# minh86/ModelCrowdNav

Measured on AMD Instinct MI355X. Metric: env-steps/sec (whole node), 5-human CrowdSim x batched envs, higher is better.
Workload: dtype f64

## Files before the change

### modelcrowdnav_amd/csrc/env_rollout_quad.hip

```cpp
#include <hip/hip_runtime.h>
#include <stdint.h>
#include "../../include/mcn.h"
#include "quad_common.hpp"
#include "env_step_params.hpp"
#include "env_common.hpp"

namespace mcn {
void note_dispatch(const char *family);
void note_rollout_form(int form);

#ifdef MCN_DIAG
#define MCN_STAMP_SLOTS 64
#define MCN_STAMP_WAVES 8192
__device__ unsigned long long g_stamps[MCN_STAMP_WAVES * MCN_STAMP_SLOTS];
#define STAMP(slot)                                                                                              \
    do {                                                                                                         \
        const int w_ = blockIdx.x * (blockDim.x >> 6) + (threadIdx.x >> 6);                                      \
        if ((threadIdx.x & 63) == 0 && (slot) < MCN_STAMP_SLOTS && w_ < MCN_STAMP_WAVES)                         \
            g_stamps[w_ * MCN_STAMP_SLOTS + (slot)] = __builtin_amdgcn_s_memrealtime();                          \
    } while (0)
#define STAMP_WHERE()                                                                                            \
    do {                                                                                                         \
        const int w_ = blockIdx.x * (blockDim.x >> 6) + (threadIdx.x >> 6);                                      \
        if ((threadIdx.x & 63) == 0 && w_ < MCN_STAMP_WAVES)                                                     \
            g_stamps[w_ * MCN_STAMP_SLOTS + 38] =                                                                \
                (unsigned long long)__builtin_amdgcn_s_getreg((4) | (0 << 6) | (31 << 11)) |                     \
                ((unsigned long long)__builtin_amdgcn_s_getreg((20) | (0 << 6) | (31 << 11)) << 32);             \
    } while (0)
int read_counts(void *dst, size_t bytes, int reset)
{
    if (bytes > sizeof(g_diag_counts)) bytes = sizeof(g_diag_counts);
    const int rc = hipMemcpyFromSymbol(dst, HIP_SYMBOL(g_diag_counts), bytes) == hipSuccess ? (int)(bytes / 4) : -1;
    if (reset) {
        void *sym = nullptr;
        if (hipGetSymbolAddress(&sym, HIP_SYMBOL(g_diag_counts)) == hipSuccess) (void)hipMemset(sym, 0, sizeof(g_diag_counts));
    }
    return rc;
}
int read_stamps(void *dst, size_t bytes)
{
    if (bytes > sizeof(g_stamps)) bytes = sizeof(g_stamps);
    return hipMemcpyFromSymbol(dst, HIP_SYMBOL(g_stamps), bytes) == hipSuccess ? (int)(bytes / 8) : -1;
}
#else
#define STAMP(slot)
#define STAMP_WHERE()
#endif

__device__ __forceinline__ int bperm_i(int byte_addr, int v) { return __builtin_amdgcn_ds_bpermute(byte_addr, v); }
__device__ __forceinline__ float bperm_f(int byte_addr, float v)
{
    return __builtin_bit_cast(float, bperm_i(byte_addr, __builtin_bit_cast(int, v)));
}
__device__ __forceinline__ double bperm_d(int byte_addr, double v)
{
    const long long b = __builtin_bit_cast(long long, v);
    const int lo = bperm_i(byte_addr, (int)b), hi = bperm_i(byte_addr, (int)(b >> 32));
    return __builtin_bit_cast(double, ((long long)hi << 32) | (unsigned int)lo);
}

template <class V>
__device__ __forceinline__ V in_vgpr(V v)
{
    asm volatile("" : "+v"(v));
    return v;
}

typedef const __attribute__((address_space(4))) StepParams *KernargPtr;
__device__ __forceinline__ KernargPtr kernarg_here()
{
    KernargPtr q = (KernargPtr)__builtin_amdgcn_kernarg_segment_ptr();
    asm volatile("" : "+s"(q));
    return q;
}

template <int NT>
struct Wg4 {
    static_assert(NT == 5, "the four-wavefront form is built for 5 humans only");
    static constexpr int EW = 8;
    static constexpr int NQ = EW * NT;
};

template <int CTRL>
__device__ __forceinline__ int dpp_i(int v) { return __builtin_amdgcn_mov_dpp(v, CTRL, 0xf, 0xf, true); }
template <int CTRL>
__device__ __forceinline__ double dpp_d(double v)
{
    const long long b = __builtin_bit_cast(long long, v);
    const int lo = dpp_i<CTRL>((int)b), hi = dpp_i<CTRL>((int)(b >> 32));
    return __builtin_bit_cast(double, ((long long)hi << 32) | (unsigned int)lo);
}
constexpr int DPP_QUAD_XOR1 = 0xB1, DPP_QUAD_XOR2 = 0x4E, DPP_ROW_HALF_MIRROR = 0x141;

template <int NT, int VIS, bool UNI>
__device__ __forceinline__ void rollout_wg4(const StepParams &p, const int T)
{
    static_assert(VIS == 0, "the four-wavefront form is built for an invisible robot only");
    constexpr int EW = Wg4<NT>::EW, NQ = Wg4<NT>::NQ;
    __shared__ float4 s_pack[NQ];
    __shared__ float2 s_res[2 * NQ], s_inv[NQ];
    __shared__ double2 s_hpos[NQ];
    __shared__ double s_hrad[NQ];
    STAMP(0);
    STAMP_WHERE();
#ifdef MCN_DIAG
    if (p.debug_noop) return;
#endif
    const int tid = threadIdx.x;
    const int role = __builtin_amdgcn_readfirstlane(tid >> 6);
    const unsigned nb_ = gridDim.x, xcd_ = blockIdx.x & 7u, idx_ = blockIdx.x >> 3;
    const unsigned qq_ = nb_ >> 3, rr__ = nb_ & 7u;
    const unsigned chunk_ = (xcd_ < rr__ ? xcd_ * (qq_ + 1) : rr__ * (qq_ + 1) + (xcd_ - rr__) * qq_) + idx_;
    const mcn_env_cfg &c = p.cfg;
    const mcn_rollout &ro = p.roll;

    if (role < 3) {
        const int lane = tid & 63, k = tid & 3, q = tid >> 2;
        const bool pop = q < NQ;
        const int ge = q / NT, h = q - ge * NT;
        const bool active = pop && (long)chunk_ * EW + ge < p.E;
        const int hi = pop ? q : 0;
        const bool cand_h = k < NT - 1;
        const int j = cand_h ? k + (k >= h ? 1 : 0) : h;
        const int ci = pop ? ge * NT + j : 0;
        const bool publish = pop && k == 0;
        const float inv_th = in_vgpr(1.0f / c.orca_time_horizon), inv_ts = in_vgpr(1.0f / (float)c.time_step);
        int rd_h = hi + NQ, rd_c = ci + NQ;
        __syncthreads();
        STAMP(1);

        for (int t = 0; t < T; ++t) {
            float4 P = s_pack[hi];
            float2 cp = *reinterpret_cast<const float2 *>(s_pack + ci);
            float2 v = s_res[rd_h], cv = s_res[rd_c];
            float2 fm = s_inv[hi];
            float orad = s_inv[ci].x;
            asm volatile("" : "+v"(P.x), "+v"(P.y), "+v"(P.z), "+v"(P.w), "+v"(cp.x), "+v"(cp.y), "+v"(v.x), "+v"(v.y),
                              "+v"(cv.x), "+v"(cv.y), "+v"(fm.x), "+v"(fm.y), "+v"(orad));
            float rx, ry;
            quad_orca_core(c, lane, k, cand_h && active, make_float4(P.x, P.y, v.x, v.y), make_float4(P.z, P.w, fm.x, fm.y),
                           make_float4(cp.x, cp.y, cv.x, cv.y), orad, inv_th, inv_ts, rx, ry);
            if (publish) s_res[(t & 1) * NQ + hi] = make_float2(rx, ry);
            rd_h = in_vgpr(hi + (t & 1) * NQ); rd_c = in_vgpr(ci + (t & 1) * NQ);
            if (t < 20) STAMP(40 + t);
            __syncthreads();
            __syncthreads();
            if (t < 37) STAMP(2 + t);
        }
    } else {
        static_assert(EW * 8 == 64, "eight lanes per env fill the wavefront");
        const double dt = in_vgpr(c.time_step);
        const bool do_reset = p.has_roll && ro.pool_hpos != nullptr;
        const int l = tid & 63;
        const int g = l >> 3, h = l & 7;
        const bool pop = h < NT;
        const int hs = g * NT + (pop ? h : 0);
        const long e = (long)chunk_ * EW + g;
        const bool active = pop && e < p.E;
        const long eb = e < p.E ? e : 0;
        const long a = eb * NT + (pop ? h : 0);
        const bool lead = active && h == 0;
        constexpr bool unicycle = UNI;
        const bool has_state = p.has_roll && ro.state != nullptr;
        const bool track = c.track_human_times && p.st.human_times != nullptr;

        double2 pos = reinterpret_cast<const double2 *>(p.st.hpos)[a];
        double2 vel = reinterpret_cast<const double2 *>(p.st.hvel)[a];
        double2 goal = reinterpret_cast<const double2 *>(p.st.hgoal)[a];
        double rad = p.st.hrad[a];
        double vpref = p.st.hvpref[a];
        double htime = p.st.human_times ? p.st.human_times[a] : 0.0;
        double hax = 0, hay = 0;
        double2 rpos = reinterpret_cast<const double2 *>(p.st.rpos)[eb];
        double2 rvel = reinterpret_cast<const double2 *>(p.st.rvel)[eb];
        double2 rgoal = reinterpret_cast<const double2 *>(p.st.rgoal)[eb];
        const double rrad = p.st.rrad[eb];
        double gtime = p.st.gtime[eb];
        double rtheta = p.st.rtheta ? p.st.rtheta[eb] : 0.0;
        mcn_roll_rec rs = {0, 0, 0, 0, 0, 0};
        if (has_state) rs = ro.state[eb];
        const double2 *act_ptr = reinterpret_cast<const double2 *>(p.actions) + eb;
        const long act_stride = in_vgpr((long)p.E);
        const double *disc_table = in_vgpr(ro.disc_table);
        const int disc_last = in_vgpr(ro.disc_len - 1);
        const bool has_theta = p.st.rtheta != nullptr;
        double2 act_next = *act_ptr;
        double o_rew = 0, o_dmin = 0;
        int o_dn = 0, o_inf = 0, o_hh = 0;
        const double k_timeout_at = in_vgpr(c.time_limit - 1);
        const double k_collision = in_vgpr(c.collision_penalty), k_success = in_vgpr(c.success_reward);
        const double k_discomfort = in_vgpr(c.discomfort_dist), k_factor = in_vgpr(c.discomfort_penalty_factor);
        const int k_stride = ro.case_stride, k_pool = ro.pool_size;
        const bool count_hh = c.count_hh != 0;
        {
            float4 A, B;
            quad_orca_operands(c, pos, vel, goal, rad, vpref, A, B);
            if (pop) {
                s_pack[hs] = make_float4(A.x, A.y, B.x, B.y); s_res[NQ + hs] = make_float2(A.z, A.w);
                s_inv[hs] = make_float2(B.z, B.w);
                s_hpos[hs] = pos; s_hrad[hs] = rad;
            }
        }
        __syncthreads();
        STAMP(1);

        for (int t = 0; t < T; ++t) {
            const double2 act = act_next;
            act_ptr += act_stride;
            if (t + 1 < T) act_next = *act_ptr;
            double ep_disc = 0;
            if (has_state) ep_disc = disc_table[rs.ep_steps < disc_last ? rs.ep_steps : disc_last];

            double2 eff = act;
            if (unicycle) {
                eff.x = act.x * cos(act.y + rtheta);
                eff.y = act.x * sin(act.y + rtheta);
            }
            double cd;
            {
                const double px = pos.x - rpos.x, py = pos.y - rpos.y;
                const double vx = vel.x - eff.x, vy = vel.y - eff.y;
                cd = p2s_origin(px, py, px + vx * dt, py + vy * dt) - rad - rrad;
            }
            cd = pop ? cd : INFINITY;
            int hh = 0;
            {
                static_assert(NT / 2 == 2, "two pairs per lane");
                double s2[2], ra[2], rb[2];
                bool near_any = false;
                const bool counted = active & count_hh;
#pragma unroll
                for (int d = 1; d <= NT / 2; ++d) {
                    const int jj = h + d >= NT ? h + d - NT : h + d;
                    const int pi = g * NT + (pop ? jj : 0);
                    const double2 ppos = s_hpos[pi];
                    const double prad = s_hrad[pi];
                    ra[d - 1] = jj > h ? rad : prad; rb[d - 1] = jj > h ? prad : rad;
                    const double dx = pos.x - ppos.x, dy = pos.y - ppos.y;
                    s2[d - 1] = dx * dx + dy * dy;
                    const double reach = ra[d - 1] + rb[d - 1] + 1e-6;
                    near_any |= counted & (s2[d - 1] < reach * reach);
                }
                if (__any(near_any)) {
                    DIAG_COUNT(2);
#pragma unroll
                    for (int d = 0; d < NT / 2; ++d)
                        hh += (counted & ((sqrt(s2[d]) - ra[d] - rb[d]) < 0)) ? 1 : 0;
                }
            }
            double dmin = cd;
            int hh_sum = hh;
            dmin = fmin(dmin, dpp_d<DPP_QUAD_XOR1>(dmin));       hh_sum += dpp_i<DPP_QUAD_XOR1>(hh_sum);
            dmin = fmin(dmin, dpp_d<DPP_QUAD_XOR2>(dmin));       hh_sum += dpp_i<DPP_QUAD_XOR2>(hh_sum);
            dmin = fmin(dmin, dpp_d<DPP_ROW_HALF_MIRROR>(dmin)); hh_sum += dpp_i<DPP_ROW_HALF_MIRROR>(hh_sum);

            double endx, endy, new_theta = rtheta, nrvx, nrvy;
            if (unicycle) {
                const double th = rtheta + act.y;
                endx = rpos.x + cos(th) * act.x * dt;
                endy = rpos.y + sin(th) * act.x * dt;
                new_theta = pymod(rtheta + act.y, 2 * M_PI);
                nrvx = act.x * cos(new_theta); nrvy = act.x * sin(new_theta);
            } else {
                endx = rpos.x + act.x * dt; endy = rpos.y + act.y * dt;
                nrvx = act.x; nrvy = act.y;
            }
            bool reaching = false;
            {
                const double gx = endx - rgoal.x, gy = endy - rgoal.y, near = rrad + 1e-6;
                if (__any(gx * gx + gy * gy < near * near)) DIAG_COUNT(3);
                if (__any(gx * gx + gy * gy < near * near)) reaching = norm2(gx, gy) < rrad;
            }
            double rew; int inf, dn;
            if (gtime >= k_timeout_at)          { rew = 0; dn = 1; inf = MCN_INFO_TIMEOUT; }
            else if (dmin < 0)                  { rew = k_collision; dn = 1; inf = MCN_INFO_COLLISION; }
            else if (reaching)                  { rew = k_success; dn = 1; inf = MCN_INFO_REACHGOAL; }
            else if (dmin < k_discomfort)       { rew = (dmin - k_discomfort) * k_factor * dt; dn = 0; inf = MCN_INFO_DANGER; }
            else                                { rew = 0; dn = 0; inf = MCN_INFO_NOTHING; }
            o_rew = rew; o_dmin = dmin; o_dn = dn; o_inf = inf; o_hh = hh_sum;
            const double t_new = gtime + dt;

            const int case_g = rs.next_case;
            if (has_state) {
                bool danger = inf == MCN_INFO_DANGER;
                if (danger) {
                    const KernargPtr kp = kernarg_here();
                    const int lim = kp->roll.danger_episodes, sf = kp->roll.danger_short_from;
                    danger = lim <= 0 || rs.fin_count < lim - ((sf > 0 && e >= sf - 1) ? 1 : 0);
                }
                rs.danger_count += danger ? 1 : 0;
                rs.danger_dist_sum = danger ? rs.danger_dist_sum + dmin : rs.danger_dist_sum;
                const double ret = rs.ep_return + ep_disc * rew;
                if (lead && dn) {
                    const int kf = rs.fin_count;
                    const KernargPtr kp = kernarg_here();
                    const int fin_slots = kp->roll.fin_slots;
                    double *fin_return = kp->roll.fin_return, *fin_time = kp->roll.fin_time;
                    uint8_t *fin_info = kp->roll.fin_info;
                    const bool keep = (fin_slots == 1) || (kf < fin_slots);
                    const long rec = (long)(fin_slots == 1 ? 0 : kf) * kp->E + e;
                    if (keep && fin_return) fin_return[rec] = ret;
                    if (keep && fin_time)   fin_time[rec] = (inf == MCN_INFO_TIMEOUT) ? kp->cfg.time_limit : t_new;
                    if (keep && fin_info)   fin_info[rec] = (uint8_t)inf;
                }
                rs.fin_count += dn;
                rs.ep_return = dn ? 0.0 : ret;
                rs.ep_steps = dn ? 0 : rs.ep_steps + 1;
                if (do_reset) {
                    int nc = rs.next_case + k_stride;
                    nc = nc >= k_pool ? nc - k_pool : nc;
                    rs.next_case = dn ? nc : rs.next_case;
                }
            }

            if (do_reset && dn) {
                const KernargPtr kp = kernarg_here();
                const double k_theta0 = kp->roll.robot_theta0;
                rpos = make_double2(kp->roll.robot_start[0], kp->roll.robot_start[1]);
                rgoal = make_double2(kp->roll.robot_goal[0], kp->roll.robot_goal[1]);
                rvel = make_double2(0, 0);
                if (has_theta) rtheta = k_theta0;
                gtime = 0;
            } else {
                rpos = make_double2(endx, endy);
                rvel = make_double2(nrvx, nrvy);
                if (unicycle) rtheta = new_theta;
                gtime = t_new;
            }

            const bool restart = do_reset && dn;
            float4 n_pack = make_float4(0, 0, 0, 0);
            float2 n_fvel = make_float2(0, 0), n_inv = make_float2(0, 0);
            if (restart) {
                DIAG_COUNT(1);
                if (active) {
                    const long pa = (long)case_g * NT + h;
                    const KernargPtr kp = kernarg_here();
                    const double2 *pool_hvel = reinterpret_cast<const double2 *>(kp->roll.pool_hvel);
                    vel = make_double2(0, 0);
                    if (pool_hvel) vel = pool_hvel[pa];
                    pos = reinterpret_cast<const double2 *>(kp->roll.pool_hpos)[pa];
                    goal = reinterpret_cast<const double2 *>(kp->roll.pool_hgoal)[pa];
                    rad = kp->roll.pool_hrad[pa];
                    vpref = kp->roll.pool_hvpref[pa];
                }
                htime = 0;
                float4 A, B;
                quad_orca_operands(c, pos, vel, goal, rad, vpref, A, B);
                n_pack = make_float4(in_vgpr(A.x), in_vgpr(A.y), in_vgpr(B.x), in_vgpr(B.y));
                n_fvel = make_float2(in_vgpr(A.z), in_vgpr(A.w));
                n_inv = make_float2(in_vgpr(B.z), in_vgpr(B.w));
            }
            const bool any_restart = __any(restart);

            if (t < 20) STAMP(40 + t);
            __syncthreads();
            float2 *vel_io = s_res + (t & 1) * NQ;
            {
                const float2 r = vel_io[hs];
                hax = (double)r.x; hay = (double)r.y;
            }
            if (!restart) {
                pos = make_double2(pos.x + hax * dt, pos.y + hay * dt);
                if (pop) s_pack[hs] = quad_orca_position_pack(pos, goal);
            }
            if (any_restart) {
                if (pop && restart) { s_pack[hs] = n_pack; vel_io[hs] = n_fvel; s_inv[hs] = n_inv; }
            }
            __syncthreads();
            if (t < 37) STAMP(2 + t);

            if (pop) s_hpos[hs] = pos;
            if (!restart) {
                vel = make_double2(hax, hay);
                if (track && htime == 0 && norm2(pos.x - goal.x, pos.y - goal.y) < rad) htime = t_new;
            }
            if (any_restart) {
                if (pop && restart) s_hrad[hs] = rad;
            }
        }

        long a2 = a, e2 = e;
        asm volatile("" : "+v"(a2), "+v"(e2));
        const KernargPtr kp = kernarg_here();
        if (active) {
            reinterpret_cast<double2 *>(kp->st.hpos)[a2] = pos;
            reinterpret_cast<double2 *>(kp->st.hvel)[a2] = vel;
            if (do_reset) {
                reinterpret_cast<double2 *>(kp->st.hgoal)[a2] = goal;
                kp->st.hrad[a2] = rad;
                kp->st.hvpref[a2] = vpref;
            }
            double *human_times = kp->st.human_times, *human_act = kp->out.human_act;
            if (human_times) human_times[a2] = htime;
            if (human_act) reinterpret_cast<double2 *>(human_act)[a2] = make_double2(hax, hay);
        }
        if (lead) {
            reinterpret_cast<double2 *>(kp->st.rpos)[e2] = rpos;
            reinterpret_cast<double2 *>(kp->st.rvel)[e2] = rvel;
            if (do_reset) reinterpret_cast<double2 *>(kp->st.rgoal)[e2] = rgoal;
            double *rth = kp->st.rtheta;
            if (rth) rth[e2] = rtheta;
            kp->st.gtime[e2] = gtime;
            store_step_rec(kp->out.rec + e2, o_rew, o_dmin, o_dn, o_inf, o_hh);
            if (has_state) kp->roll.state[e2] = rs;
        }
    }
    STAMP(39);
}

template <int NT, int VIS, bool UNI>
__global__ __launch_bounds__(256, 2) void env_rollout_wg4_kernel(const StepParams p, const int T)
{
    rollout_wg4<NT, VIS, UNI>(p, T);
}

template <int NT, int VIS, bool UNI, bool SPLIT>
__global__ __launch_bounds__(SPLIT ? 128 : 64, SPLIT ? 3 : 1) void env_rollout_quad_kernel(const StepParams p, const int T)
{
    __shared__ double2 s_hpos[16], s_hvel[16], s_rpos[16], s_rvel[16];
    __shared__ double s_hrad[16];
    __shared__ int s_dn[16], s_case[16];
    STAMP(0);
    STAMP_WHERE();
#ifdef MCN_DIAG
    if (p.debug_noop) return;
#endif
    const int role = SPLIT ? (int)(threadIdx.x >> 6) : -1;
    const bool do_orca = role != 1, do_pair = role != 0;
    constexpr int NC = NT - 1 + VIS;
    constexpr int LPE = 4 * NT;
    constexpr int G = 64 / LPE;
    static_assert(NC >= 0 && NC <= 4, "quad kernel handles at most 4 ORCA neighbours");
    const int lane = threadIdx.x & 63;
    const int g = lane / LPE;
    const int r = lane - g * LPE;
    const int h = r >> 2, k = r & 3;
#ifndef MCN_QUAD_XCD
#define MCN_QUAD_XCD 1
#endif
    const unsigned nb_ = gridDim.x, xcd_ = blockIdx.x & 7u, idx_ = blockIdx.x >> 3;
    const unsigned qq_ = nb_ >> 3, rr__ = nb_ & 7u;
    const unsigned chunk_ = MCN_QUAD_XCD ? (xcd_ < rr__ ? xcd_ * (qq_ + 1) : rr__ * (qq_ + 1) + (xcd_ - rr__) * qq_) + idx_
                                         : blockIdx.x;
    const long e = (long)chunk_ * G + g;
    const bool active = (g < G) && (e < p.E);
    const long eb = active ? e : 0;
    const long a = eb * NT + h;
    const int gi = g < G ? g : 0;
    const int hi = g < G ? g * NT + h : 0;
    const mcn_env_cfg &c = p.cfg;
    const mcn_rollout &ro = p.roll;
    const double dt = in_vgpr(c.time_step);
    const bool lead = active && r == 0 && do_pair;
    const bool hlead = active && k == 0 && do_orca;
    constexpr bool unicycle = UNI;
    const bool has_state = p.has_roll && ro.state != nullptr;
    const bool do_reset = p.has_roll && ro.pool_hpos != nullptr;
    const bool track = c.track_human_times && p.st.human_times != nullptr;

    double2 pos = reinterpret_cast<const double2 *>(p.st.hpos)[a];
    double2 vel = reinterpret_cast<const double2 *>(p.st.hvel)[a];
    double2 goal = reinterpret_cast<const double2 *>(p.st.hgoal)[a];
    double rad = p.st.hrad[a];
    double vpref = p.st.hvpref[a];
    double htime = p.st.human_times ? p.st.human_times[a] : 0.0;
    double2 rpos = reinterpret_cast<const double2 *>(p.st.rpos)[eb];
    double2 rvel = reinterpret_cast<const double2 *>(p.st.rvel)[eb];
    double2 rgoal = reinterpret_cast<const double2 *>(p.st.rgoal)[eb];
    const double rrad = p.st.rrad[eb];
    double gtime = p.st.gtime[eb];
    double rtheta = p.st.rtheta ? p.st.rtheta[eb] : 0.0;
    mcn_roll_rec rs = {0, 0, 0, 0, 0, 0};
    if (has_state) rs = ro.state[eb];

    const bool cand_h = k < NT - 1;
    const bool cand_r = VIS && (k == NT - 1);
    const int j = cand_h ? k + (k >= h ? 1 : 0) : h;
    const int l0 = lane - r;
    const int src = ((l0 + 4 * j) & 63) << 2;

    const double2 *act_ptr = reinterpret_cast<const double2 *>(p.actions) + eb;
    const long act_stride = in_vgpr((long)p.E);
    const double *disc_table = in_vgpr(ro.disc_table);
    const int disc_last = in_vgpr(ro.disc_len - 1);
    const bool has_theta = p.st.rtheta != nullptr;
    double2 act_next = *act_ptr;
    double o_rew = 0, o_dmin = 0;
    int o_dn = 0, o_inf = 0, o_hh = 0;
    double hax = 0, hay = 0;
    const float inv_th = in_vgpr(1.0f / c.orca_time_horizon), inv_ts = in_vgpr(1.0f / (float)c.time_step);
    STAMP(1);

    for (int t = 0; t < T; ++t) {
        const double2 act = act_next;
        act_ptr += act_stride;
        if (do_pair && t + 1 < T) act_next = *act_ptr;
        double ep_disc = 0;
        if (do_pair && has_state) ep_disc = disc_table[rs.ep_steps < disc_last ? rs.ep_steps : disc_last];

        double2 cpos;
        cpos.x = bperm_d(src, pos.x);
        cpos.y = bperm_d(src, pos.y);
        double crd = bperm_d(src, rad);
        float cvx = bperm_f(src, (float)vel.x), cvy = bperm_f(src, (float)vel.y);
        if (cand_r) { cpos = rpos; crd = rrad; }

        int dn = 0, case_g = 0;
        double t_new = 0;

        if (do_orca) {
            if (cand_r) { cvx = (float)rvel.x; cvy = (float)rvel.y; }
            float rx, ry;
            quad_orca_velocity(c, lane, k, (cand_h || cand_r) && active, pos, vel, goal, rad, vpref,
                               make_float4((float)cpos.x, (float)cpos.y, cvx, cvy), crd, inv_th, inv_ts, rx, ry);
            hax = (double)rx; hay = (double)ry;
        }

        if (do_pair) {
            double2 eff = act;
            if (unicycle) {
                eff.x = act.x * cos(act.y + rtheta);
                eff.y = act.x * sin(act.y + rtheta);
            }
            double cd;
            {
                const double px = pos.x - rpos.x, py = pos.y - rpos.y;
                const double vx = vel.x - eff.x, vy = vel.y - eff.y;
                cd = p2s_origin(px, py, px + vx * dt, py + vy * dt) - rad - rrad;
            }
            int hh = 0;
            {
                const double dx = pos.x - cpos.x, dy = pos.y - cpos.y;
                const bool counted = active & (c.count_hh != 0) & cand_h & (j > h);
                const double s2 = dx * dx + dy * dy, reach = rad + crd + 1e-6;
                if (__any(counted & (s2 < reach * reach))) DIAG_COUNT(2);
                if (__any(counted & (s2 < reach * reach)))
                    hh = (counted & ((sqrt(s2) - rad - crd) < 0)) ? 1 : 0;
            }
            hh += __builtin_amdgcn_update_dpp(0, hh, 0xB1, 0xf, 0xf, false);
            hh += __builtin_amdgcn_update_dpp(0, hh, 0x4E, 0xf, 0xf, false);
            double dmin = INFINITY;
            int hh_sum = 0;
#pragma unroll
            for (int q = 0; q < NT; ++q) {
                const int s = (l0 + 4 * q) & 63;
                dmin = fmin(dmin, __shfl(cd, s));
                hh_sum += __shfl(hh, s);
            }

            double endx, endy, new_theta = rtheta, nrvx, nrvy;
            if (unicycle) {
                const double th = rtheta + act.y;
                endx = rpos.x + cos(th) * act.x * dt;
                endy = rpos.y + sin(th) * act.x * dt;
                new_theta = pymod(rtheta + act.y, 2 * M_PI);
                nrvx = act.x * cos(new_theta); nrvy = act.x * sin(new_theta);
            } else {
                endx = rpos.x + act.x * dt; endy = rpos.y + act.y * dt;
                nrvx = act.x; nrvy = act.y;
            }
            bool reaching = false;
            {
                const double gx = endx - rgoal.x, gy = endy - rgoal.y, near = rrad + 1e-6;
                if (__any(gx * gx + gy * gy < near * near)) DIAG_COUNT(3);
                if (__any(gx * gx + gy * gy < near * near)) reaching = norm2(gx, gy) < rrad;
            }
            const KernargPtr kc = kernarg_here();
            const double k_time_limit = kc->cfg.time_limit, k_timeout_at = k_time_limit - 1;
            const double k_collision = kc->cfg.collision_penalty, k_success = kc->cfg.success_reward;
            const double k_discomfort = kc->cfg.discomfort_dist, k_factor = kc->cfg.discomfort_penalty_factor;
            double rew; int inf;
            if (gtime >= k_timeout_at)          { rew = 0; dn = 1; inf = MCN_INFO_TIMEOUT; }
            else if (dmin < 0)                  { rew = k_collision; dn = 1; inf = MCN_INFO_COLLISION; }
            else if (reaching)                  { rew = k_success; dn = 1; inf = MCN_INFO_REACHGOAL; }
            else if (dmin < k_discomfort)       { rew = (dmin - k_discomfort) * k_factor * dt; dn = 0; inf = MCN_INFO_DANGER; }
            else                                { rew = 0; dn = 0; inf = MCN_INFO_NOTHING; }
            o_rew = rew; o_dmin = dmin; o_dn = dn; o_inf = inf; o_hh = hh_sum;
            t_new = gtime + dt;

            case_g = rs.next_case;
            if (has_state) {
                bool danger = inf == MCN_INFO_DANGER;
                if (danger) {
                    const KernargPtr kp = kernarg_here();
                    const int lim = kp->roll.danger_episodes, sf = kp->roll.danger_short_from;
                    danger = lim <= 0 || rs.fin_count < lim - ((sf > 0 && e >= sf - 1) ? 1 : 0);
                }
                rs.danger_count += danger ? 1 : 0;
                rs.danger_dist_sum = danger ? rs.danger_dist_sum + dmin : rs.danger_dist_sum;
                const double ret = rs.ep_return + ep_disc * rew;
                if (lead && dn) {
                    const int kf = rs.fin_count;
                    const KernargPtr kp = kernarg_here();
                    const int fin_slots = kp->roll.fin_slots;
                    double *fin_return = kp->roll.fin_return, *fin_time = kp->roll.fin_time;
                    uint8_t *fin_info = kp->roll.fin_info;
                    const bool keep = (fin_slots == 1) || (kf < fin_slots);
                    const long rec = (long)(fin_slots == 1 ? 0 : kf) * kp->E + e;
                    if (keep && fin_return) fin_return[rec] = ret;
                    if (keep && fin_time)   fin_time[rec] = (inf == MCN_INFO_TIMEOUT) ? k_time_limit : t_new;
                    if (keep && fin_info)   fin_info[rec] = (uint8_t)inf;
                }
                rs.fin_count += dn;
                rs.ep_return = dn ? 0.0 : ret;
                rs.ep_steps = dn ? 0 : rs.ep_steps + 1;
                if (do_reset) {
                    const int k_stride = kc->roll.case_stride, k_pool = kc->roll.pool_size;
                    int nc = rs.next_case + k_stride;
                    nc = nc >= k_pool ? nc - k_pool : nc;
                    rs.next_case = dn ? nc : rs.next_case;
                }
            }

            if (do_reset && dn) {
                const KernargPtr kp = kernarg_here();
                const double k_theta0 = kp->roll.robot_theta0;
                rpos = make_double2(kp->roll.robot_start[0], kp->roll.robot_start[1]);
                rgoal = make_double2(kp->roll.robot_goal[0], kp->roll.robot_goal[1]);
                rvel = make_double2(0, 0);
                if (has_theta) rtheta = k_theta0;
                gtime = 0;
            } else {
                rpos = make_double2(endx, endy);
                rvel = make_double2(nrvx, nrvy);
                if (unicycle) rtheta = new_theta;
                gtime = t_new;
            }
        }

        if (SPLIT) {
            if (lead) {
                s_dn[gi] = dn; s_case[gi] = case_g;
                if (VIS) { s_rpos[gi] = rpos; s_rvel[gi] = rvel; }
            }
            __syncthreads();
            if (role == 0) {
                dn = s_dn[gi]; case_g = s_case[gi];
                if (VIS) { rpos = s_rpos[gi]; rvel = s_rvel[gi]; }
            }
        }

        if (do_orca) {
            if (do_reset && dn) {
                DIAG_COUNT(1);
                if (active) {
                    const long pa = (long)case_g * NT + h;
                    const KernargPtr kp = kernarg_here();
                    const double2 *pool_hvel = reinterpret_cast<const double2 *>(kp->roll.pool_hvel);
                    pos = reinterpret_cast<const double2 *>(kp->roll.pool_hpos)[pa];
                    goal = reinterpret_cast<const double2 *>(kp->roll.pool_hgoal)[pa];
                    rad = kp->roll.pool_hrad[pa];
                    vpref = kp->roll.pool_hvpref[pa];
                    vel = pool_hvel ? pool_hvel[pa] : make_double2(0, 0);
                }
                htime = 0;
            } else {
                pos = make_double2(pos.x + hax * dt, pos.y + hay * dt);
                vel = make_double2(hax, hay);
                if (track && htime == 0 && norm2(pos.x - goal.x, pos.y - goal.y) < rad) htime = SPLIT ? gtime + dt : t_new;
            }
        }
        if (SPLIT) {
            if (role == 0) gtime = (do_reset && dn) ? 0.0 : gtime + dt;
            if (hlead) { s_hpos[hi] = pos; s_hvel[hi] = vel; s_hrad[hi] = rad; }
            __syncthreads();
            if (role == 1) { pos = s_hpos[hi]; vel = s_hvel[hi]; rad = s_hrad[hi]; }
        }
        if (t < 37) STAMP(2 + t);
    }

    {
        long a2 = a, e2 = e;
        asm volatile("" : "+v"(a2), "+v"(e2));
        const KernargPtr kp = kernarg_here();
        if (hlead) {
            reinterpret_cast<double2 *>(kp->st.hpos)[a2] = pos;
            reinterpret_cast<double2 *>(kp->st.hvel)[a2] = vel;
            if (do_reset) {
                reinterpret_cast<double2 *>(kp->st.hgoal)[a2] = goal;
                kp->st.hrad[a2] = rad;
                kp->st.hvpref[a2] = vpref;
            }
            double *human_times = kp->st.human_times, *human_act = kp->out.human_act;
            if (human_times) human_times[a2] = htime;
            if (human_act) reinterpret_cast<double2 *>(human_act)[a2] = make_double2(hax, hay);
        }
        if (lead) {
            reinterpret_cast<double2 *>(kp->st.rpos)[e2] = rpos;
            reinterpret_cast<double2 *>(kp->st.rvel)[e2] = rvel;
            if (do_reset) reinterpret_cast<double2 *>(kp->st.rgoal)[e2] = rgoal;
            double *rth = kp->st.rtheta;
            if (rth) rth[e2] = rtheta;
            kp->st.gtime[e2] = gtime;
            store_step_rec(kp->out.rec + e2, o_rew, o_dmin, o_dn, o_inf, o_hh);
            if (has_state) kp->roll.state[e2] = rs;
        }
    }
    STAMP(39);
}

template <int NT, int VIS, bool UNI>
static void launch_rollout_kin(const StepParams &p, int T, int blocks, hipStream_t stream)
{
    if constexpr (NT == 5 && VIS == 0) {
        if (p.quad_split == 2) {
            constexpr int EW = Wg4<NT>::EW;
            hipLaunchKernelGGL((env_rollout_wg4_kernel<NT, VIS, UNI>), dim3((p.E + EW - 1) / EW), dim3(256), 0, stream, p, T);
            note_rollout_form(2);
            return;
        }
    }
    if (p.quad_split)
        hipLaunchKernelGGL((env_rollout_quad_kernel<NT, VIS, UNI, true>), dim3(blocks), dim3(128), 0, stream, p, T);
    else
        hipLaunchKernelGGL((env_rollout_quad_kernel<NT, VIS, UNI, false>), dim3(blocks), dim3(64), 0, stream, p, T);
    note_rollout_form(p.quad_split ? 1 : 0);
}

template <int NT, int VIS>
static void launch_rollout_one(const StepParams &p, int T, hipStream_t stream)
{
    constexpr int G = 64 / (4 * NT);
    const int blocks = (p.E + G - 1) / G;
    if (p.cfg.robot_kinematics == MCN_KIN_UNICYCLE)
        launch_rollout_kin<NT, VIS, true>(p, T, blocks, stream);
    else
        launch_rollout_kin<NT, VIS, false>(p, T, blocks, stream);
}

bool launch_env_rollout_quad(const StepParams &p, int T, hipStream_t stream)
{
    if (p.cfg.human_policy != MCN_HUMANS_ORCA || p.cfg.orca_max_neighbors < 4 || !p.update) return false;
    const int vis = p.cfg.robot_visible ? 1 : 0;
    const int nc = p.N - 1 + vis;
    if (nc > 4 || p.N < 1) return false;
    switch (p.N * 2 + vis) {
        case 2:  launch_rollout_one<1, 0>(p, T, stream); break;
        case 3:  launch_rollout_one<1, 1>(p, T, stream); break;
        case 4:  launch_rollout_one<2, 0>(p, T, stream); break;
        case 5:  launch_rollout_one<2, 1>(p, T, stream); break;
        case 6:  launch_rollout_one<3, 0>(p, T, stream); break;
        case 7:  launch_rollout_one<3, 1>(p, T, stream); break;
        case 8:  launch_rollout_one<4, 0>(p, T, stream); break;
        case 9:  launch_rollout_one<4, 1>(p, T, stream); break;
        case 10: launch_rollout_one<5, 0>(p, T, stream); break;
        default: return false;
    }
    note_dispatch("env_rollout_quad_kernel");
    return true;
}

}
```

### modelcrowdnav_amd/csrc/mcn_api.hip

```cpp
#include <hip/hip_runtime.h>
#include <string.h>
#include <stdlib.h>
#include <math.h>
#include <mutex>
#include "../../include/mcn.h"

#include "env_step_params.hpp"
#include "lp3_queue.hpp"

namespace mcn {
int launch_env_step(const StepParams &p, hipStream_t stream);
bool launch_env_rollout_quad(const StepParams &p, int T, hipStream_t stream);
bool launch_env_step_loop(const StepParams &p, int T, hipStream_t stream);
bool launch_env_step_loop_sf(const StepParams &p, int T, hipStream_t stream);
int launch_env_step_loop_orca(const StepParams &p, const ClosedLoop &cl, int T, hipStream_t stream);
int launch_scenario_pool(const mcn_scenario_cfg &c, uint64_t seed, int64_t first_case, int P, int N, double *hpos,
                         double *hgoal, double *hrad, double *hvpref, hipStream_t stream);
struct SarlParams;
long sarl_workspace_float4s(int E, int N, int A);
int launch_mlp_world(const mcn_mlp_world_net *net, const double *hpos, const double *hvel, double *out_vel, int E, int N,
                     hipStream_t stream);
int launch_attn_world(const mcn_attn_world_net *net, const double *hpos, const double *hvel, const int32_t *hcount,
                      void *workspace, double *out_vel, int E, int N, hipStream_t stream);
long attn_world_workspace_float4s(int E, int N);
int launch_sarl_c(const mcn_sarl_net *net, const mcn_env_state *st, const double *actions, int A, double dt,
                  double gamma_pow, int kinematics, void *workspace, double *values, int32_t *best, double *best_val,
                  float *attention, const double *next_hpos, const double *next_hvel, const double *reward_in,
                  double *action_out, double epsilon, unsigned long long seed, int E, int N, const float *om_init,
                  hipStream_t stream);
int launch_sarl_om(const mcn_env_state *st, double dt, const double *next_hpos, const double *next_hvel,
                   double cell_size, const float *w_om, const float *b_om, float *om, float *init, int E, int N,
                   hipStream_t stream);
int launch_lstm_rl(const mcn_lstm_rl_net *net, const mcn_env_state *st, const double *actions, int A, double dt,
                   double gamma_pow, int kinematics, double *values, int32_t *best, double *best_val, int32_t *order,
                   const double *next_hpos, const double *next_hvel, const double *reward_in, double *action_out,
                   double epsilon, unsigned long long seed, int E, int N, hipStream_t stream);
int launch_cadrl(const mcn_cadrl_net *net, const mcn_env_state *st, const double *actions, int A, double dt,
                 double gamma_pow, int kinematics, double *values, int32_t *best, double *best_val,
                 const double *next_hpos, const double *next_hvel, const double *reward_in, double *action_out,
                 double epsilon, unsigned long long seed, int E, int N, hipStream_t stream);
int launch_lstm_rl_order(const double *hpos, const double *rpos, const int32_t *hcount, int32_t *order, int E, int N,
                         hipStream_t stream);
#ifdef MCN_DIAG
int read_pool_clock(void *dst, size_t bytes);
int read_sarl_phases(void *dst, size_t bytes, int reset);
#endif
int launch_sgan(const mcn_sgan_net *net, double *hist, int push_slot, int oldest, const double *cur_pos,
                const float *noise, const int32_t *hcount, void *workspace, double *out_vel, float *out_rel,
                double time_step, int E, int N, hipStream_t stream);
int launch_sgan_predict(const mcn_sgan_net *net, const double *hist, int oldest, const float *noise, int K, int T,
                        const int32_t *hcount, void *workspace, float *out_rel, double *out_pos, int E, int N,
                        hipStream_t stream);
int launch_orca_batch(const float *self, const float *others, const int32_t *n_other, float *out,
                      int B, int M, float neighbor_dist, int max_neighbors, float time_horizon, float time_step,
                      hipStream_t stream);
int launch_orca_finish(const mcn_env_state &st, float *sim_vel, const uint8_t *select, int max_steps, int32_t *steps,
                       float *traj, double time_step, float neighbor_dist, int max_neighbors, float time_horizon,
                       int E, int N, hipStream_t stream);
#ifdef MCN_DIAG
int read_stamps(void *dst, size_t bytes);
int read_counts(void *dst, size_t bytes, int reset);
#endif
}

static mcn_tuning g_tuning;
static bool g_tuning_init = false;
static std::mutex g_tuning_mu;
static int env_or(const char *name, int dflt)
{
    const char *v = getenv(name);
    return v ? atoi(v) : dflt;
}
static mcn_tuning tuning_from_env()
{
    mcn_tuning t;
    memset(&t, 0, sizeof(t));
    t.force_generic = env_or("MCN_FORCE_GENERIC", 0);
    t.quad_max_envs = env_or("MCN_QUAD_MAX_ENVS", -1);
    t.quad_split = env_or("MCN_QUAD_SPLIT", -1);
    t.rollout_fused = env_or("MCN_ROLLOUT_FUSED", -1);
    t.rollout_split = env_or("MCN_ROLLOUT_SPLIT", -1);
    t.step_block = env_or("MCN_STEP_BLOCK", -1);
    t.pair_stream = env_or("MCN_PAIR_STREAM", -1);
    t.lp3_defer = env_or("MCN_LP3_DEFER", -1);
    t.sarl_x3 = env_or("MCN_SARL_X3", -1);
    return t;
}
static mcn_tuning tuning()
{
    std::lock_guard<std::mutex> lock(g_tuning_mu);
    if (!g_tuning_init) { g_tuning = tuning_from_env(); g_tuning_init = true; }
    return g_tuning;
}

namespace mcn { bool tuning_sarl_x3() { return tuning().sarl_x3 != 0; } }

static uint16_t bf16_rne(float x)
{
    uint32_t u;
    memcpy(&u, &x, 4);
    if ((u & 0x7fffffffu) > 0x7f800000u) return (uint16_t)((u >> 16) | 0x40);
    u += 0x7fffu + ((u >> 16) & 1u);
    return (uint16_t)(u >> 16);
}
static float bf16_to_f32(uint16_t h) { const uint32_t u = (uint32_t)h << 16; float f; memcpy(&f, &u, 4); return f; }

int64_t mcn_pack_x3_bytes(int32_t NT, int32_t KT)
{
    if (NT <= 0 || KT <= 0) return 0;
    return (int64_t)NT * ((KT + 1) / 2) * 3 * 64 * 8 * 2;
}

int mcn_pack_x3(const float *wfrag, int32_t NT, int32_t KT, void *x3_out)
{
    if (!wfrag || !x3_out || NT <= 0 || KT <= 0) return MCN_EINVAL;
    const int KB = (KT + 1) / 2;
    uint16_t *out = reinterpret_cast<uint16_t *>(x3_out);
    for (int n = 0; n < NT; ++n)
        for (int m = 0; m < KB; ++m)
            for (int lane = 0; lane < 64; ++lane)
                for (int s = 0; s < 8; ++s) {
                    const int t = 2 * m + (s >> 2);
                    const float w = t < KT ? wfrag[(((size_t)n * KT + t) * 64 + lane) * 4 + (s & 3)] : 0.0f;
                    const uint16_t hi = bf16_rne(w);
                    const float r1 = w - bf16_to_f32(hi);
                    const uint16_t mid = bf16_rne(r1);
                    const float r2 = r1 - bf16_to_f32(mid);
                    const size_t at = (((size_t)n * KB + m) * 3 * 64 + lane) * 8 + s;
                    out[at] = hi; out[at + 64 * 8] = mid; out[at + 2 * 64 * 8] = bf16_rne(r2);
                }
    return MCN_OK;
}

static thread_local const char *g_last_dispatch = "";
namespace mcn { void note_dispatch(const char *family) { g_last_dispatch = family; } }
const char *mcn_last_dispatch(void) { return g_last_dispatch; }
static thread_local int32_t g_last_rollout_form = -1;
namespace mcn { void note_rollout_form(int form) { g_last_rollout_form = form; } }
int32_t mcn_last_rollout_form(void) { return g_last_rollout_form; }

int32_t mcn_abi_version(void) { return MCN_ABI_VERSION; }
int64_t mcn_sizeof(int32_t which)
{
    switch (which) {
        case MCN_SIZEOF_ENV_CFG: return sizeof(mcn_env_cfg);
        case MCN_SIZEOF_ENV_STATE: return sizeof(mcn_env_state);
        case MCN_SIZEOF_ENV_OUT: return sizeof(mcn_env_out);
        case MCN_SIZEOF_ROLLOUT: return sizeof(mcn_rollout);
        case MCN_SIZEOF_TUNING: return sizeof(mcn_tuning);
        case MCN_SIZEOF_STEP_REC: return sizeof(mcn_step_rec);
        case MCN_SIZEOF_ROLL_REC: return sizeof(mcn_roll_rec);
        case MCN_SIZEOF_SARL_NET: return sizeof(mcn_sarl_net);
        case MCN_SIZEOF_SGAN_NET: return sizeof(mcn_sgan_net);
        case MCN_SIZEOF_SCENARIO_CFG: return sizeof(mcn_scenario_cfg);
        case MCN_SIZEOF_MLP_WORLD_NET: return sizeof(mcn_mlp_world_net);
        case MCN_SIZEOF_ATTN_WORLD_NET: return sizeof(mcn_attn_world_net);
        case MCN_SIZEOF_SARL_X3: return sizeof(mcn_sarl_x3);
        case MCN_SIZEOF_LSTM_RL_NET: return sizeof(mcn_lstm_rl_net);
        case MCN_SIZEOF_CADRL_NET: return sizeof(mcn_cadrl_net);
        default: return -1;
    }
}

static int fill_step_params(mcn::StepParams &p, const mcn_env_cfg *cfg, const mcn_env_state *st, const double *actions,
                            const double *given_v, const mcn_env_out *out, const mcn_rollout *roll,
                            int32_t E, int32_t N, int32_t update, bool social_force = false, bool needs_actions = true)
{
    if (!cfg || !st || !out || (needs_actions && !actions)) return MCN_EINVAL;
    if (E <= 0 || N <= 0 || N > MCN_MAX_HUMANS) return MCN_EINVAL;
    if (!st->hpos || !st->hvel || !st->hgoal || !st->hrad || !st->hvpref || !st->rpos || !st->rvel || !st->rgoal ||
        !st->rrad || !st->gtime) return MCN_EINVAL;
    if (cfg->robot_kinematics == MCN_KIN_UNICYCLE && !st->rtheta) return MCN_EINVAL;
    if (!out->rec) return MCN_EINVAL;
    if (!update && (!out->nobs_pos || !out->nobs_vel)) return MCN_EINVAL;
    if (cfg->human_policy == MCN_HUMANS_GIVEN && !given_v) return MCN_EINVAL;
    if (social_force) {
        if (cfg->human_policy != MCN_HUMANS_SOCIALFORCE) return MCN_EINVAL;
    } else if (cfg->human_policy < MCN_HUMANS_ORCA || cfg->human_policy > MCN_HUMANS_GIVEN) return MCN_EINVAL;
    if (cfg->orca_max_neighbors < 0 || cfg->orca_max_neighbors > MCN_MAX_LINES) return MCN_EINVAL;
    if (!(cfg->time_step > 0)) return MCN_EINVAL;
    if (roll) {
        if (roll->state && (!roll->disc_table || roll->disc_len <= 0 || roll->fin_slots < 1)) return MCN_EINVAL;
        if (roll->pool_hpos && !roll->state) return MCN_EINVAL;
        if (roll->pool_hpos && (!roll->pool_hgoal || !roll->pool_hrad || !roll->pool_hvpref || roll->pool_size <= 0)) return MCN_EINVAL;
        if (roll->pool_hpos && (roll->case_stride < 0 || roll->case_stride >= roll->pool_size)) return MCN_EINVAL;
    }
    memset(&p, 0, sizeof(p));
    p.cfg = *cfg; p.st = *st; p.out = *out;
    if (roll) { p.roll = *roll; p.has_roll = 1; }
    p.actions = actions; p.given_v = given_v;
    p.E = E; p.N = N; p.G = 64 / N; p.update = update ? 1 : 0;
    int ncand = N - 1 + (cfg->robot_visible ? 1 : 0);
    int nl = ncand < cfg->orca_max_neighbors ? ncand : cfg->orca_max_neighbors;
    if (cfg->human_policy != MCN_HUMANS_ORCA) nl = 0;
    p.nl_cap = nl;
    const mcn_tuning tu = tuning();
    p.force_generic = tu.force_generic > 0 ? 1 : 0;
    p.pair_stream = tu.pair_stream;
    p.step_block = tu.step_block;
    p.lp3_defer = tu.lp3_defer;
#ifdef MCN_DIAG
    p.debug_noop = tu.diag_noop;
#endif
    const int envs_per_wave = 64 / (4 * N);
    const long quad_waves = envs_per_wave > 0 ? ((long)E + envs_per_wave - 1) / envs_per_wave : (1L << 40);
    p.quad_max_envs = tu.quad_max_envs >= 0 ? tu.quad_max_envs : (quad_waves <= 2800 ? E : 0);
    p.quad_split = tu.quad_split >= 0 ? tu.quad_split : (quad_waves <= 1400 ? 1 : 0);
    return MCN_OK;
}

extern "C" {

#ifdef MCN_DIAG
const char *mcn_version(void) { return "modelcrowdnav_amd 0.4 (gfx950) DIAGNOSTIC BUILD (time stamps)"; }
#else
const char *mcn_version(void) { return "modelcrowdnav_amd 0.4 (gfx950)"; }
#endif

int mcn_set_tuning(const mcn_tuning *t)
{
    std::lock_guard<std::mutex> lock(g_tuning_mu);
    if (!t) { g_tuning = tuning_from_env(); g_tuning_init = true; return MCN_OK; }
    if (t->quad_split > 1 || t->rollout_fused > 1 || t->rollout_split > 2 || t->pair_stream > 3 || t->force_generic < 0 || t->force_generic > 1) return MCN_EINVAL;
    if (t->quad_max_envs < -1 || t->quad_split < -1 || t->rollout_fused < -1 || t->rollout_split < -1 || t->pair_stream < -1) return MCN_EINVAL;
    if (t->step_block != -1 && t->step_block != 64 && t->step_block != 256) return MCN_EINVAL;
    if (t->lp3_defer < -1 || t->lp3_defer > 1) return MCN_EINVAL;
    if (t->sarl_x3 < -1 || t->sarl_x3 > 1) return MCN_EINVAL;
#ifndef MCN_DIAG
    if (t->diag_noop) return MCN_EINVAL;
#endif
    g_tuning = *t;
    g_tuning_init = true;
    return MCN_OK;
}

int mcn_get_tuning(mcn_tuning *t)
{
    if (!t) return MCN_EINVAL;
    *t = tuning();
    return MCN_OK;
}

int64_t mcn_env_lp3_queue_bytes(int32_t E, int32_t N)
{
    if (E <= 0 || N < 2 || N > 10) return 0;
    return mcn::lp3_queue_bytes(E, N, N < MCN_MAX_LINES ? N : MCN_MAX_LINES);
}

int mcn_env_step(const mcn_env_cfg *cfg, const mcn_env_state *st, const double *actions,
                 const double *given_v, const mcn_env_out *out, const mcn_rollout *roll,
                 int32_t E, int32_t N, int32_t update, void *stream)
{
    mcn::StepParams p;
    const int rc = fill_step_params(p, cfg, st, actions, given_v, out, roll, E, N, update);
    if (rc != MCN_OK) return rc;
    return mcn::launch_env_step(p, (hipStream_t)stream);
}

int mcn_env_rollout(const mcn_env_cfg *cfg, const mcn_env_state *st, const double *actions, int32_t T,
                    const mcn_env_out *out, const mcn_rollout *roll, int32_t E, int32_t N, void *stream)
{
    if (T <= 0) return MCN_EINVAL;
    mcn::StepParams p;
    const int rc = fill_step_params(p, cfg, st, actions, nullptr, out, roll, E, N, 1);
    if (rc != MCN_OK) return rc;
    const mcn_tuning tu = tuning();
    const int envs_per_wave = 64 / (4 * N) > 0 ? 64 / (4 * N) : 1;
    const long waves = ((long)E + envs_per_wave - 1) / envs_per_wave;
    const bool fused = tu.rollout_fused >= 0 ? tu.rollout_fused != 0 : waves <= 14000;
    const int step_split = p.quad_split;
    const long wg4 = ((long)E + 7) / 8;
    const bool wg4_wins = N == 5 && !cfg->robot_visible &&
                          (cfg->robot_kinematics == MCN_KIN_UNICYCLE ? wg4 >= 8 && wg4 <= 1024
                                                                     : (wg4 >= 128 && wg4 <= 512) || (wg4 >= 768 && wg4 <= 1024));
    p.quad_split = tu.rollout_split >= 0 ? tu.rollout_split : wg4_wins ? 2 : (waves <= 1536 ? 1 : 0);
    mcn::note_rollout_form(-1);
    if (fused && !p.force_generic && mcn::launch_env_rollout_quad(p, T, (hipStream_t)stream))
        return hipGetLastError() == hipSuccess ? MCN_OK : MCN_ELAUNCH;
    p.quad_split = step_split;
    if (tu.rollout_fused != 0 && T > 1 && mcn::launch_env_step_loop(p, T, (hipStream_t)stream))
        return hipGetLastError() == hipSuccess ? MCN_OK : MCN_ELAUNCH;
    for (int32_t t = 0; t < T; ++t) {
        p.actions = actions + (size_t)t * E * 2;
        const int r = mcn::launch_env_step(p, (hipStream_t)stream);
        if (r != MCN_OK) return r;
    }
    return MCN_OK;
}

int mcn_env_rollout_orca(const mcn_env_cfg *cfg, const mcn_env_state *st, double robot_safety_space,
                         float neighbor_dist, int32_t max_neighbors, float time_horizon, int32_t T,
                         const mcn_env_out *out, const mcn_rollout *roll, double *tr_robot, double *tr_humans,
                         double *tr_hrad, double *tr_action, mcn_step_rec *tr_rec, double *tr_human_act,
                         int32_t E, int32_t N, void *stream)
{
    if (!cfg || !st || !out || T < 1) return MCN_EINVAL;
    if (max_neighbors < 0 || max_neighbors > MCN_MAX_LINES) return MCN_EINVAL;
    if (!(time_horizon > 0) || !(cfg->time_step > 0) || !((float)cfg->time_step > 0)) return MCN_EINVAL;
    if (!isfinite(robot_safety_space)) return MCN_EINVAL;
    if (cfg->robot_kinematics != MCN_KIN_HOLONOMIC) return MCN_EINVAL;
    if (cfg->human_policy != MCN_HUMANS_ORCA && cfg->human_policy != MCN_HUMANS_LINEAR) return MCN_EINVAL;
    if (!st->rvpref) return MCN_EINVAL;
    mcn::StepParams p;
    const int rc = fill_step_params(p, cfg, st, nullptr, nullptr, out, roll, E, N, 1, false, false);
    if (rc != MCN_OK) return rc;
    mcn::ClosedLoop cl;
    memset(&cl, 0, sizeof(cl));
    cl.safety_space = robot_safety_space;
    cl.neighbor_dist = neighbor_dist; cl.time_horizon = time_horizon; cl.max_neighbors = max_neighbors;
    cl.tr_robot = tr_robot; cl.tr_humans = tr_humans; cl.tr_hrad = tr_hrad; cl.tr_action = tr_action;
    cl.tr_rec = tr_rec; cl.tr_human_act = tr_human_act;
    return mcn::launch_env_step_loop_orca(p, cl, T, (hipStream_t)stream);
}

static bool sf_params_ok(double strength, double range, double relaxation_rate)
{
    return isfinite(strength) && isfinite(range) && isfinite(relaxation_rate) && strength >= 0 && range > 0 &&
           relaxation_rate >= 0;
}

int mcn_env_step_sf(const mcn_env_cfg *cfg, double strength, double range, double relaxation_rate,
                    const mcn_env_state *st, const double *actions, const mcn_env_out *out,
                    const mcn_rollout *roll, int32_t E, int32_t N, int32_t update, void *stream)
{
    if (!sf_params_ok(strength, range, relaxation_rate)) return MCN_EINVAL;
    mcn::StepParams p;
    const int rc = fill_step_params(p, cfg, st, actions, nullptr, out, roll, E, N, update, true);
    if (rc != MCN_OK) return rc;
    p.sf_strength = strength; p.sf_range = range; p.sf_relaxation_rate = relaxation_rate;
    return mcn::launch_env_step(p, (hipStream_t)stream);
}

int mcn_env_rollout_sf(const mcn_env_cfg *cfg, double strength, double range, double relaxation_rate,
                       const mcn_env_state *st, const double *actions, int32_t T, const mcn_env_out *out,
                       const mcn_rollout *roll, int32_t E, int32_t N, void *stream)
{
    if (T <= 0 || !sf_params_ok(strength, range, relaxation_rate)) return MCN_EINVAL;
    mcn::StepParams p;
    const int rc = fill_step_params(p, cfg, st, actions, nullptr, out, roll, E, N, 1, true);
    if (rc != MCN_OK) return rc;
    p.sf_strength = strength; p.sf_range = range; p.sf_relaxation_rate = relaxation_rate;
    if (tuning().rollout_fused != 0 && T > 1 && mcn::launch_env_step_loop_sf(p, T, (hipStream_t)stream))
        return hipGetLastError() == hipSuccess ? MCN_OK : MCN_ELAUNCH;
    for (int32_t t = 0; t < T; ++t) {
        p.actions = actions + (size_t)t * E * 2;
        const int r = mcn::launch_env_step(p, (hipStream_t)stream);
        if (r != MCN_OK) return r;
    }
    return MCN_OK;
}

int mcn_scenario_pool(const mcn_scenario_cfg *cfg, uint64_t seed, int64_t first_case, int32_t P, int32_t N,
                      double *hpos, double *hgoal, double *hrad, double *hvpref, void *stream)
{
    if (!cfg || !hpos || !hgoal || !hrad || !hvpref) return MCN_EINVAL;
    if (P <= 0 || N <= 0 || N > MCN_MAX_HUMANS) return MCN_EINVAL;
    if (cfg->rule != MCN_RULE_CIRCLE && cfg->rule != MCN_RULE_SQUARE) return MCN_EINVAL;
    if (!(cfg->circle_radius > 0) || !(cfg->square_width > 0) || !(cfg->human_radius > 0)) return MCN_EINVAL;
    return mcn::launch_scenario_pool(*cfg, seed, first_case, P, N, hpos, hgoal, hrad, hvpref, (hipStream_t)stream);
}

int mcn_orca_batch(const float *self, const float *others, const int32_t *n_other, float *out,
                   int32_t B, int32_t M, float neighbor_dist, int32_t max_neighbors,
                   float time_horizon, float time_step, void *stream)
{
    if (!self || !n_other || !out || B <= 0 || M < 0 || M > MCN_MAX_HUMANS) return MCN_EINVAL;
    if (M > 0 && !others) return MCN_EINVAL;
    if (max_neighbors < 0 || max_neighbors > MCN_MAX_LINES) return MCN_EINVAL;
    if (!(time_horizon > 0) || !(time_step > 0)) return MCN_EINVAL;
    return mcn::launch_orca_batch(self, others, n_other, out, B, M, neighbor_dist, max_neighbors,
                                  time_horizon, time_step, (hipStream_t)stream);
}

int mcn_orca_finish(const mcn_env_state *st, float *sim_vel, const uint8_t *select, int32_t max_steps, int32_t *steps,
                    float *traj, double time_step, float neighbor_dist, int32_t max_neighbors, float time_horizon,
                    int32_t E, int32_t N, void *stream)
{
    if (!st || !sim_vel || !steps || max_steps < 1 || E <= 0 || N < 1 || N > MCN_MAX_HUMANS) return MCN_EINVAL;
    if (!st->hpos || !st->hgoal || !st->hrad || !st->hvpref || !st->rpos || !st->rgoal || !st->rrad || !st->rvpref ||
        !st->gtime || !st->human_times) return MCN_EINVAL;
    if (max_neighbors < 0 || max_neighbors > MCN_MAX_LINES) return MCN_EINVAL;
    if (!(time_horizon > 0) || !(time_step > 0) || !((float)time_step > 0)) return MCN_EINVAL;
    return mcn::launch_orca_finish(*st, sim_vel, select, max_steps, steps, traj, time_step, neighbor_dist, max_neighbors,
                                   time_horizon, E, N, (hipStream_t)stream);
}

int mcn_pack_linear(const float *weight, const float *bias, int32_t nout, int32_t kin,
                    const int32_t *kmap, int32_t KT, const int32_t *omap, int32_t NT,
                    float *wfrag_out, float *bfrag_out)
{
    if (!weight || !kmap || !wfrag_out || nout <= 0 || kin <= 0 || KT <= 0 || NT <= 0) return MCN_EINVAL;
    if (!omap && NT != (nout + 15) / 16) return MCN_EINVAL;
    auto orow = [&](int n, int slot) { return omap ? omap[n * 16 + slot] : 16 * n + slot; };
    for (int n = 0; n < NT; ++n)
        for (int slot = 0; slot < 16; ++slot)
            if (orow(n, slot) >= nout) { if (omap) return MCN_EINVAL; }
    for (int n = 0; n < NT; ++n)
        for (int t = 0; t < KT; ++t)
            for (int lane = 0; lane < 64; ++lane)
                for (int r = 0; r < 4; ++r) {
                    const int row = orow(n, lane & 15);
                    const int col = kmap[t * 16 + 4 * (lane >> 4) + r];
                    float v = 0.0f;
                    if (row >= 0 && row < nout && col >= 0) {
                        if (col >= kin) return MCN_EINVAL;
                        v = weight[(size_t)row * kin + col];
                    }
                    wfrag_out[(((size_t)n * KT + t) * 64 + lane) * 4 + r] = v;
                }
    if (bfrag_out)
        for (int n = 0; n < NT; ++n)
            for (int lane = 0; lane < 64; ++lane)
                for (int r = 0; r < 4; ++r) {
                    const int row = orow(n, 4 * (lane >> 4) + r);
                    bfrag_out[((size_t)n * 64 + lane) * 4 + r] = (bias && row >= 0 && row < nout) ? bias[row] : 0.0f;
                }
    return MCN_OK;
}

int64_t mcn_sarl_workspace_bytes(int32_t E, int32_t N, int32_t A)
{
    if (E <= 0 || N <= 0 || A <= 0) return 0;
    return (int64_t)mcn::sarl_workspace_float4s(E, N, A) * 16;
}

static bool lookahead_common_ok(const void *net, size_t net_bytes, const mcn_env_state *st, const double *actions,
                                int32_t A, double time_step, int32_t kinematics, const double *values,
                                const double *next_hpos, const double *next_hvel, double epsilon, int32_t E, int32_t N)
{
    if (!net || !st || !actions || !values) return false;
    if (!(epsilon >= 0.0 && epsilon <= 1.0)) return false;
    if (E <= 0 || N <= 0 || N > MCN_MAX_HUMANS || A <= 0) return false;
    if (!st->hpos || !st->hvel || !st->hrad || !st->rpos || !st->rgoal || !st->rrad || !st->rvpref) return false;
    if (kinematics == MCN_KIN_UNICYCLE && !st->rtheta) return false;
    if ((next_hpos == nullptr) != (next_hvel == nullptr)) return false;
    const float *const *fp = reinterpret_cast<const float *const *>(net);
    for (size_t k = 0; k < net_bytes / sizeof(float *); ++k)
        if (!fp[k]) return false;
    return time_step > 0;
}

static int sarl_lookahead_impl(const mcn_sarl_net *net, const mcn_env_state *st, const double *actions, int32_t A,
                               double time_step, double gamma_pow, int32_t kinematics, void *workspace,
                               double *values, int32_t *best, double *best_val, float *attention,
                               const double *next_hpos, const double *next_hvel, const double *rewards,
                               double *action_out, double epsilon, uint64_t seed, int32_t E, int32_t N,
                               const float *om_init, void *stream)
{
    if (!lookahead_common_ok(net, sizeof(*net), st, actions, A, time_step, kinematics, values, next_hpos, next_hvel,
                             epsilon, E, N))
        return MCN_EINVAL;
    if (!workspace) return MCN_EINVAL;
    if (action_out && !best) return MCN_EINVAL;
    if (best && !best_val) return MCN_EINVAL;
    return mcn::launch_sarl_c(net, st, actions, A, time_step, gamma_pow, kinematics, workspace, values, best,
                              best_val, attention, next_hpos, next_hvel, rewards, action_out, epsilon,
                              (unsigned long long)seed, E, N, om_init, (hipStream_t)stream);
}

int mcn_sarl_lookahead(const mcn_sarl_net *net, const mcn_env_state *st, const double *actions, int32_t A,
                       double time_step, double gamma_pow, int32_t kinematics, void *workspace,
                       double *values, int32_t *best, double *best_val, float *attention,
                       int32_t E, int32_t N, void *stream)
{
    return sarl_lookahead_impl(net, st, actions, A, time_step, gamma_pow, kinematics, workspace, values, best, best_val,
                               attention, nullptr, nullptr, nullptr, nullptr, 0.0, 0, E, N, nullptr, stream);
}

int mcn_sarl_lookahead_env(const mcn_sarl_net *net, const mcn_env_state *st, const double *actions, int32_t A,
                           double time_step, double gamma_pow, int32_t kinematics, void *workspace,
                           double *values, int32_t *best, double *best_val, float *attention,
                           const double *next_hpos, const double *next_hvel, const double *rewards,
                           int32_t E, int32_t N, void *stream)
{
    if (!next_hpos || !next_hvel || !rewards) return MCN_EINVAL;
    return sarl_lookahead_impl(net, st, actions, A, time_step, gamma_pow, kinematics, workspace, values, best, best_val,
                               attention, next_hpos, next_hvel, rewards, nullptr, 0.0, 0, E, N, nullptr, stream);
}

int mcn_sarl_predict(const mcn_sarl_net *net, const mcn_env_state *st, const double *actions, int32_t A,
                     double time_step, double gamma_pow, int32_t kinematics, void *workspace,
                     double *values, int32_t *best, double *best_val, float *attention,
                     const double *next_hpos, const double *next_hvel, const double *rewards,
                     double *action_out, double epsilon, uint64_t seed, int32_t E, int32_t N, void *stream)
{
    if (!best || !action_out) return MCN_EINVAL;
    if ((next_hpos == nullptr) != (rewards == nullptr)) return MCN_EINVAL;
    return sarl_lookahead_impl(net, st, actions, A, time_step, gamma_pow, kinematics, workspace, values, best, best_val,
                               attention, next_hpos, next_hvel, rewards, action_out, epsilon, seed, E, N, nullptr, stream);
}

int mcn_sarl_om_prepare(const mcn_env_state *st, double time_step, const double *next_hpos, const double *next_hvel,
                        double cell_size, const float *w_om, const float *b_om, float *om, float *init,
                        int32_t E, int32_t N, void *stream)
{
    if (!st || !om) return MCN_EINVAL;
    if (E <= 0 || N <= 0 || N > MCN_MAX_HUMANS) return MCN_EINVAL;
    if (!st->hpos || !st->hvel) return MCN_EINVAL;
    if ((next_hpos == nullptr) != (next_hvel == nullptr)) return MCN_EINVAL;
    if (!(time_step >= 0.0) || !(cell_size > 0.0)) return MCN_EINVAL;
    if ((w_om == nullptr) != (init == nullptr) || (b_om == nullptr) != (init == nullptr)) return MCN_EINVAL;
    return mcn::launch_sarl_om(st, time_step, next_hpos, next_hvel, cell_size, w_om, b_om, om, init, E, N,
                               (hipStream_t)stream);
}

int mcn_sarl_predict_om(const mcn_sarl_net *net, const mcn_env_state *st, const double *actions, int32_t A,
                        double time_step, double gamma_pow, int32_t kinematics, void *workspace,
                        double *values, int32_t *best, double *best_val, float *attention,
                        const double *next_hpos, const double *next_hvel, const double *rewards,
                        double *action_out, double epsilon, uint64_t seed, const float *om_init,
                        int32_t E, int32_t N, void *stream)
{
    if (!best || !action_out || !om_init) return MCN_EINVAL;
    if ((next_hpos == nullptr) != (rewards == nullptr)) return MCN_EINVAL;
    return sarl_lookahead_impl(net, st, actions, A, time_step, gamma_pow, kinematics, workspace, values, best, best_val,
                               attention, next_hpos, next_hvel, rewards, action_out, epsilon, seed, E, N, om_init, stream);
}

static int lookahead_args_ok(const void *net, size_t net_bytes, const mcn_env_state *st, const double *actions, int32_t A,
                             double time_step, int32_t kinematics, const double *values, const int32_t *best,
                             const double *best_val, const double *next_hpos, const double *next_hvel,
                             const double *rewards, const double *action_out, double epsilon, int32_t E, int32_t N)
{
    if (!lookahead_common_ok(net, net_bytes, st, actions, A, time_step, kinematics, values, next_hpos, next_hvel, epsilon, E, N))
        return 0;
    if (!best || !best_val || !action_out) return 0;
    if (kinematics != MCN_KIN_HOLONOMIC && kinematics != MCN_KIN_UNICYCLE) return 0;
    return (next_hpos == nullptr) == (rewards == nullptr);
}

int mcn_lstm_rl_predict(const mcn_lstm_rl_net *net, const mcn_env_state *st, const double *actions, int32_t A,
                        double time_step, double gamma_pow, int32_t kinematics,
                        double *values, int32_t *best, double *best_val, int32_t *order,
                        const double *next_hpos, const double *next_hvel, const double *rewards,
                        double *action_out, double epsilon, uint64_t seed, int32_t E, int32_t N, void *stream)
{
    if (!lookahead_args_ok(net, sizeof(*net), st, actions, A, time_step, kinematics, values, best, best_val, next_hpos,
                           next_hvel, rewards, action_out, epsilon, E, N))
        return MCN_EINVAL;
    return mcn::launch_lstm_rl(net, st, actions, A, time_step, gamma_pow, kinematics, values, best, best_val, order,
                               next_hpos, next_hvel, rewards, action_out, epsilon, (unsigned long long)seed, E, N,
                               (hipStream_t)stream);
}

int mcn_lstm_rl_order(const mcn_env_state *st, int32_t *order, int32_t E, int32_t N, void *stream)
{
    if (!st || !order || !st->hpos || !st->rpos || E <= 0 || N <= 0 || N > MCN_MAX_HUMANS) return MCN_EINVAL;
    return mcn::launch_lstm_rl_order(st->hpos, st->rpos, st->hcount, order, E, N, (hipStream_t)stream);
}

int mcn_cadrl_predict(const mcn_cadrl_net *net, const mcn_env_state *st, const double *actions, int32_t A,
                      double time_step, double gamma_pow, int32_t kinematics,
                      double *values, int32_t *best, double *best_val,
                      const double *next_hpos, const double *next_hvel, const double *rewards,
                      double *action_out, double epsilon, uint64_t seed, int32_t E, int32_t N, void *stream)
{
    if (!lookahead_args_ok(net, sizeof(*net), st, actions, A, time_step, kinematics, values, best, best_val, next_hpos,
                           next_hvel, rewards, action_out, epsilon, E, N))
        return MCN_EINVAL;
    return mcn::launch_cadrl(net, st, actions, A, time_step, gamma_pow, kinematics, values, best, best_val, next_hpos,
                             next_hvel, rewards, action_out, epsilon, (unsigned long long)seed, E, N, (hipStream_t)stream);
}

int mcn_mlp_world_step(const mcn_mlp_world_net *net, const double *hpos, const double *hvel, double *out_vel,
                       int32_t E, int32_t N, void *stream)
{
    if (!net || !hpos || !hvel || !out_vel || E <= 0 || N <= 0 || N > 10) return MCN_EINVAL;
    const float *const *fp = reinterpret_cast<const float *const *>(net);
    for (int k = 0; k < 8; ++k)
        if (!fp[k]) return MCN_EINVAL;
    return mcn::launch_mlp_world(net, hpos, hvel, out_vel, E, N, (hipStream_t)stream);
}

int64_t mcn_attn_world_workspace_bytes(int32_t E, int32_t N)
{
    if (E <= 0 || N <= 0) return 0;
    return (int64_t)mcn::attn_world_workspace_float4s(E, N) * 16;
}

int mcn_attn_world_step(const mcn_attn_world_net *net, const double *hpos, const double *hvel, const int32_t *hcount,
                        void *workspace, double *out_vel, int32_t E, int32_t N, void *stream)
{
    if (!net || !hpos || !hvel || !workspace || !out_vel || E <= 0 || N <= 0 || N > MCN_MAX_HUMANS) return MCN_EINVAL;
    const float *const *fp = reinterpret_cast<const float *const *>(net);
    for (size_t k = 0; k < sizeof(mcn_attn_world_net) / sizeof(float *); ++k)
        if (!fp[k]) return MCN_EINVAL;
    return mcn::launch_attn_world(net, hpos, hvel, hcount, workspace, out_vel, E, N, (hipStream_t)stream);
}

int64_t mcn_sgan_workspace_bytes(int32_t E, int32_t N)
{
    if (E <= 0 || N <= 0) return 0;
    return (int64_t)E * N * (32 + 4 + 8) * 4;
}

int mcn_sgan_step(const mcn_sgan_net *net, double *hist, int32_t push_slot, int32_t oldest, const double *cur_pos,
                  const float *noise, const int32_t *hcount, void *workspace, double *out_vel, float *out_rel,
                  double time_step, int32_t E, int32_t N, void *stream)
{
    if (!net || !hist || !noise || !workspace || !out_vel) return MCN_EINVAL;
    if (E <= 0 || N <= 0 || N > MCN_MAX_HUMANS) return MCN_EINVAL;
    if (push_slot < 0 || push_slot > 7 || oldest < 0 || oldest > 7 || !(time_step > 0)) return MCN_EINVAL;
    const float *const *fp = reinterpret_cast<const float *const *>(net);
    for (int k = 0; k < 14; ++k) {
        const bool pool_only = (k >= 2 && k < 6);
        if (!fp[k] && !(pool_only && !net->pooling)) return MCN_EINVAL;
    }
    return mcn::launch_sgan(net, hist, push_slot, oldest, cur_pos, noise, hcount, workspace, out_vel, out_rel,
                            time_step, E, N, (hipStream_t)stream);
}

int mcn_sgan_predict(const mcn_sgan_net *net, const double *hist, int32_t oldest, const float *noise, int32_t K, int32_t T,
                     const int32_t *hcount, void *workspace, float *out_rel, double *out_pos, int32_t E, int32_t N,
                     void *stream)
{
    if (!net || !hist || !noise || !workspace || !out_rel) return MCN_EINVAL;
    if (K < 1 || K > 65535 || T < 1) return MCN_EINVAL;
    if (E <= 0 || N <= 0 || N > MCN_MAX_HUMANS || oldest < 0 || oldest > 7) return MCN_EINVAL;
    const float *const *fp = reinterpret_cast<const float *const *>(net);
    for (int k = 0; k < 14; ++k) {
        const bool pool_only = (k >= 2 && k < 6);
        if (!fp[k] && !(pool_only && !net->pooling)) return MCN_EINVAL;
    }
    return mcn::launch_sgan_predict(net, hist, oldest, noise, K, T, hcount, workspace, out_rel, out_pos, E, N,
                                    (hipStream_t)stream);
}

#ifdef MCN_DIAG
int mcn_debug_pool_clock(void *dst_host, int64_t bytes) { return mcn::read_pool_clock(dst_host, (size_t)bytes); }
int mcn_debug_sarl_phases(void *dst_host, int64_t bytes, int32_t reset) { return mcn::read_sarl_phases(dst_host, (size_t)bytes, reset); }
int mcn_debug_stamps(void *dst_host, int64_t bytes) { return mcn::read_stamps(dst_host, (size_t)bytes); }
int mcn_debug_counts(void *dst_host, int64_t bytes, int reset) { return mcn::read_counts(dst_host, (size_t)bytes, reset); }
#endif

}
```

### modelcrowdnav_amd/csrc/orca_static.hpp

```cpp
#pragma once
#include <hip/hip_runtime.h>
#include "orca_device.hpp"
#include "fast_f32.hpp"

namespace mcn {

#ifndef MCN_STATIC_LINE
#define MCN_STATIC_LINE orca_line_select
#endif

__device__ __forceinline__ float4 orca_line_merged(float px, float py, float vx, float vy, float radius, float4 o,
                                                   float orad, float inv_th, float inv_ts)
{
        const float rpx = o.x - px, rpy = o.y - py;
    const float rvx = vx - o.z, rvy = vy - o.w;
    const float dist_sq = dot2(rpx, rpy, rpx, rpy);
    const float cr = radius + orad;
    const float cr_sq = cr * cr;
    const bool apart = dist_sq > cr_sq;
    const float inv = apart ? inv_th : inv_ts;
    const float wx = rvx - inv * rpx, wy = rvy - inv * rpy;
    const float wl_sq = dot2(wx, wy, wx, wy);
    const float dp1 = dot2(wx, wy, rpx, rpy);
    float dx, dy, ux, uy;
    if (!apart || (dp1 < 0.0f && dp1 * dp1 > cr_sq * wl_sq)) {
        const float wl = sqrtf(wl_sq);
        const float iw = 1.0f / wl;
        const float uwx = wx * iw, uwy = wy * iw;
        dx = uwy; dy = -uwx;
        const float s = cr * inv - wl;
        ux = s * uwx; uy = s * uwy;
    } else {
        const float leg = sqrtf(dist_sq - cr_sq);
        const float id = 1.0f / dist_sq;
        if (det2(rpx, rpy, wx, wy) > 0.0f) {
            dx = (rpx * leg - rpy * cr) * id;
            dy = (rpx * cr + rpy * leg) * id;
        } else {
            dx = -((rpx * leg + rpy * cr) * id);
            dy = -((-rpx * cr + rpy * leg) * id);
        }
        const float dp2 = dot2(rvx, rvy, dx, dy);
        ux = dp2 * dx - rvx; uy = dp2 * dy - rvy;
    }
    return make_float4(vx + 0.5f * ux, vy + 0.5f * uy, dx, dy);
}

__device__ __forceinline__ float4 orca_u_dir(float px, float py, float vx, float vy, float radius, float4 o,
                                             float orad, float inv_th, float inv_ts, bool used = true)
{
    const float rpx = o.x - px, rpy = o.y - py;
    const float rvx = vx - o.z, rvy = vy - o.w;
    const float dist_sq = dot2(rpx, rpy, rpx, rpy);
    const float cr = radius + orad;
    const float cr_sq = cr * cr;
    const bool apart = dist_sq > cr_sq;
    const float inv = apart ? inv_th : inv_ts;
    const float wx = rvx - inv * rpx, wy = rvy - inv * rpy;
    const float wl_sq = dot2(wx, wy, wx, wy);
    const float dp1 = dot2(wx, wy, rpx, rpy);
    const bool circle = !apart | ((dp1 < 0.0f) & (dp1 * dp1 > cr_sq * wl_sq));
    const float leg_sq = dist_sq - cr_sq;
    float wl, iw, leg, id;
#if MCN_FAST_F32
    const unsigned long long m_circle = ~lanes(apart) | (lanes(dp1 < 0.0f) & lanes(dp1 * dp1 > cr_sq * wl_sq));
    const unsigned long long m_used = lanes(used);
    const unsigned long long m_w = __builtin_amdgcn_ballot_w64(sqrt5_ok(wl_sq));
    const unsigned long long m_l = __builtin_amdgcn_ballot_w64(sqrt5_ok(leg_sq)) & __builtin_amdgcn_ballot_w64(dist_sq < 0x1p126f);
    if ((m_used & ~((m_circle & m_w) | (~m_circle & m_l))) == 0) {
        wl = sqrt5(wl_sq); iw = rcp3(wl); leg = sqrt5(leg_sq); id = rcp3(dist_sq);
    } else
#endif
    {
        wl = sqrtf(wl_sq); iw = 1.0f / wl; leg = sqrtf(leg_sq); id = 1.0f / dist_sq;
    }
    const float uwx = wx * iw, uwy = wy * iw;
    const float sc = cr * inv - wl;
    const float cux = sc * uwx, cuy = sc * uwy;
    const bool left = det2(rpx, rpy, wx, wy) > 0.0f;
    const float lx = (rpx * leg - rpy * cr) * id, ly = (rpx * cr + rpy * leg) * id;
    const float rx = -((rpx * leg + rpy * cr) * id), ry = -((-rpx * cr + rpy * leg) * id);
    const float gx = left ? lx : rx, gy = left ? ly : ry;
    const float dp2 = dot2(rvx, rvy, gx, gy);
    const float lux = dp2 * gx - rvx, luy = dp2 * gy - rvy;
    const float dx = circle ? uwy : gx, dy = circle ? -uwx : gy;
    const float ux = circle ? cux : lux, uy = circle ? cuy : luy;
    return make_float4(ux, uy, dx, dy);
}

__device__ __forceinline__ float4 orca_line_select(float px, float py, float vx, float vy, float radius, float4 o,
                                                   float orad, float inv_th, float inv_ts, bool used = true)
{
    const float4 ud = orca_u_dir(px, py, vx, vy, radius, o, orad, inv_th, inv_ts, used);
    return make_float4(vx + 0.5f * ud.x, vy + 0.5f * ud.y, ud.z, ud.w);
}

template <int NO, int NL, bool DIR = false>
__device__ __forceinline__ bool lp1_s(const float4 (&L)[NL], float radius, float optx, float opty, float &rx, float &ry)
{
    const float4 ln = L[NO];
    const float dp = dot2(ln.x, ln.y, ln.z, ln.w);
    const float disc = dp * dp + radius * radius - dot2(ln.x, ln.y, ln.x, ln.y);
    if (disc < 0.0f) return false;
    const float sq = sqrt_f32(disc);
    float tl = -dp - sq;
    float tr = -dp + sq;
    bool ok = true;
#pragma unroll
    for (int i = 0; i < NO; ++i) {
        const float4 li = L[i];
        const float den = det2(ln.z, ln.w, li.z, li.w);
        const float num = det2(li.z, li.w, ln.x - li.x, ln.y - li.y);
        const float t = num / den;
        const bool par = fabsf(den) <= kRvoEps;
        const float ntr = fminf(tr, t), ntl = fmaxf(tl, t);
        tr = (!par & (den >= 0.0f)) ? ntr : tr;
        tl = (!par & !(den >= 0.0f)) ? ntl : tl;
        ok = ok & !(par & (num < 0.0f)) & !(!par & (tl > tr));
    }
    if (!ok) return false;
    float t;
    if constexpr (DIR) {
        t = (dot2(optx, opty, ln.z, ln.w) > 0.0f) ? tr : tl;
    } else {
        t = dot2(ln.z, ln.w, optx - ln.x, opty - ln.y);
        if (t < tl) t = tl; else if (t > tr) t = tr;
    }
    rx = ln.x + t * ln.z;
    ry = ln.y + t * ln.w;
    return true;
}

template <int I, int NL, bool DIR = false>
struct Lp2Step {
    static __device__ __forceinline__ void run(const float4 (&L)[NL], int n, float radius, float optx, float opty,
                                               float &rx, float &ry, int &fail)
    {
        if constexpr (I < NL) {
            if (I < n && fail == n) {
                const float4 li = L[I];
                if (det2(li.z, li.w, li.x - rx, li.y - ry) > 0.0f) {
                    float nx = rx, ny = ry;
                    if (lp1_s<I, NL, DIR>(L, radius, optx, opty, nx, ny)) { rx = nx; ry = ny; }
                    else fail = I;
                }
            }
            Lp2Step<I + 1, NL, DIR>::run(L, n, radius, optx, opty, rx, ry, fail);
        }
    }
};

template <int I, int NL>
struct Lp3Step {
    static __device__ __forceinline__ void run(const float4 (&L)[NL], int n, int begin, float radius, float &rx, float &ry,
                                               float &dist)
    {
        if constexpr (I < NL) {
            if (I >= begin && I < n) {
                const float4 li = L[I];
                if (det2(li.z, li.w, li.x - rx, li.y - ry) > dist) {
                    constexpr int NP = I > 0 ? I : 1;
                    float4 P[NP];
                    int m = 0;
#pragma unroll
                    for (int jj = 0; jj < I; ++jj) {
                        const float4 lj = L[jj];
                        const float dt = det2(li.z, li.w, lj.z, lj.w);
                        float qx, qy;
                        bool skip = false;
                        if (fabsf(dt) <= kRvoEps) {
                            if (dot2(li.z, li.w, lj.z, lj.w) > 0.0f) skip = true;
                            qx = 0.5f * (li.x + lj.x); qy = 0.5f * (li.y + lj.y);
                        } else {
                            const float sc = det2(lj.z, lj.w, li.x - lj.x, li.y - lj.y) / dt;
                            qx = li.x + sc * li.z; qy = li.y + sc * li.w;
                        }
                        const float ddx = lj.z - li.z, ddy = lj.w - li.w;
                        const float inv = rcp_sqrt_f32(dot2(ddx, ddy, ddx, ddy));
                        const float4 q = make_float4(qx, qy, ddx * inv, ddy * inv);
#pragma unroll
                        for (int sl = 0; sl < NP; ++sl)
                            if (!skip && sl == m) P[sl] = q;
                        m += skip ? 0 : 1;
                    }
                    const float kx = rx, ky = ry;
                    const float ox = -li.w, oy = li.z;
                    rx = radius * ox; ry = radius * oy;
                    int fail = m;
                    if constexpr (I > 0) Lp2Step<0, NP, true>::run(P, m, radius, ox, oy, rx, ry, fail);
                    if (fail < m) { rx = kx; ry = ky; }
                    dist = det2(li.z, li.w, li.x - rx, li.y - ry);
                }
            }
            Lp3Step<I + 1, NL>::run(L, n, begin, radius, rx, ry, dist);
        }
    }
};

constexpr int kLp3StaticMax = 10;

template <int NC>
__device__ __forceinline__ void orca_solve_static(float4 (&cpv)[NC > 0 ? NC : 1], float (&crad)[NC > 0 ? NC : 1],
                                                  float px, float py, float vx, float vy, float radius,
                                                  float max_speed, float prefx, float prefy, float neighbor_dist,
                                                  int max_neighbors, float time_horizon, float time_step,
                                                  float &outx, float &outy)
{
    constexpr int NL = NC < kMaxLines ? (NC > 0 ? NC : 1) : kMaxLines;
    const float range_sq = neighbor_dist * neighbor_dist;
    float d[NC > 0 ? NC : 1];
    int nin = 0;
#pragma unroll
    for (int c = 0; c < NC; ++c) {
        const float ddx = px - cpv[c].x, ddy = py - cpv[c].y;
        const float dd = dot2(ddx, ddy, ddx, ddy);
        const bool in = dd < range_sq;
        d[c] = in ? dd : INFINITY;
        nin += in;
    }
#pragma unroll
    for (int i = 1; i < NC; ++i) {
#pragma unroll
        for (int j = i; j >= 1; --j) {
            const bool sw = d[j] < d[j - 1];
            const float td = sw ? d[j - 1] : d[j];       d[j - 1] = sw ? d[j] : d[j - 1];       d[j] = td;
            const float tr = sw ? crad[j - 1] : crad[j]; crad[j - 1] = sw ? crad[j] : crad[j - 1]; crad[j] = tr;
            const float4 a = cpv[j - 1], b = cpv[j];
            cpv[j - 1] = make_float4(sw ? b.x : a.x, sw ? b.y : a.y, sw ? b.z : a.z, sw ? b.w : a.w);
            cpv[j]     = make_float4(sw ? a.x : b.x, sw ? a.y : b.y, sw ? a.z : b.z, sw ? a.w : b.w);
        }
    }
    int nl = nin < max_neighbors ? nin : max_neighbors;
    if (nl > NL) nl = NL;

    const float inv_th = 1.0f / time_horizon;
    const float inv_ts = 1.0f / time_step;
    float4 L[NL];
#pragma unroll
    for (int k = 0; k < NL; ++k) {
        if (k < NC) {
            L[k] = MCN_STATIC_LINE(px, py, vx, vy, radius, cpv[k], crad[k], inv_th, inv_ts);
        } else {
            L[k] = make_float4(0, 0, 1, 0);
        }
    }

    float rx, ry;
    if (dot2(prefx, prefy, prefx, prefy) > max_speed * max_speed) {
        const float inv = rcp_sqrt_f32(dot2(prefx, prefy, prefx, prefy));
        rx = max_speed * (prefx * inv); ry = max_speed * (prefy * inv);
    } else {
        rx = prefx; ry = prefy;
    }
    int fail = nl;
    Lp2Step<0, NL>::run(L, nl, max_speed, prefx, prefy, rx, ry, fail);

    if constexpr (NL <= kLp3StaticMax) {
        if (fail < nl) {
            float dist = 0.0f;
            Lp3Step<0, NL>::run(L, nl, fail, max_speed, rx, ry, dist);
        }
    } else if (fail < nl) {
        float4 buf[NL];
#pragma unroll
        for (int k = 0; k < NL; ++k) buf[k] = L[k];
        PrivLines PL{buf};
        lp3(PL, nl, fail, max_speed, rx, ry);
    }
    outx = rx; outy = ry;
}

template <int NC>
__device__ __forceinline__ void orca_sort_lp2(float4 (&Lnat)[NC > 0 ? NC : 1], float (&dd)[NC > 0 ? NC : 1],
                                              float max_speed, float prefx, float prefy, float neighbor_dist,
                                              int max_neighbors, float &rx, float &ry, int &fail, int &nl)
{
    constexpr int NL = NC > 0 ? NC : 1;
    static_assert(NC <= kMaxLines, "more candidates than line slots: the tail of the sorted list would be lost");
    const float range_sq = neighbor_dist * neighbor_dist;
    float d[NL];
    int nin = 0;
#pragma unroll
    for (int c = 0; c < NC; ++c) {
        const bool in = dd[c] < range_sq;
        d[c] = in ? dd[c] : INFINITY;
        nin += in;
    }
#pragma unroll
    for (int i = 1; i < NC; ++i) {
#pragma unroll
        for (int j = i; j >= 1; --j) {
            const bool sw = d[j] < d[j - 1];
            const float td = sw ? d[j - 1] : d[j];       d[j - 1] = sw ? d[j] : d[j - 1];       d[j] = td;
            const float4 a = Lnat[j - 1], b = Lnat[j];
            Lnat[j - 1] = make_float4(sw ? b.x : a.x, sw ? b.y : a.y, sw ? b.z : a.z, sw ? b.w : a.w);
            Lnat[j]     = make_float4(sw ? a.x : b.x, sw ? a.y : b.y, sw ? a.z : b.z, sw ? a.w : b.w);
        }
    }
    nl = nin < max_neighbors ? nin : max_neighbors;
    if (nl > NL) nl = NL;
    if (dot2(prefx, prefy, prefx, prefy) > max_speed * max_speed) {
        const float inv = rcp_sqrt_f32(dot2(prefx, prefy, prefx, prefy));
        rx = max_speed * (prefx * inv); ry = max_speed * (prefy * inv);
    } else {
        rx = prefx; ry = prefy;
    }
    fail = nl;
    Lp2Step<0, NL>::run(Lnat, nl, max_speed, prefx, prefy, rx, ry, fail);
}

template <int NL>
__device__ __forceinline__ void lp3_static(const float4 (&L)[NL], int nl, int fail, float max_speed, float &rx, float &ry)
{
    if (fail < nl) {
        float dist = 0.0f;
        Lp3Step<0, NL>::run(L, nl, fail, max_speed, rx, ry, dist);
    }
}

template <int NC>
__device__ __forceinline__ void orca_solve_static_lines(float4 (&Lnat)[NC > 0 ? NC : 1], float (&dd)[NC > 0 ? NC : 1],
                                                        float max_speed, float prefx, float prefy, float neighbor_dist,
                                                        int max_neighbors, float &outx, float &outy)
{
    int nl, fail;
    orca_sort_lp2<NC>(Lnat, dd, max_speed, prefx, prefy, neighbor_dist, max_neighbors, outx, outy, fail, nl);
    lp3_static<(NC > 0 ? NC : 1)>(Lnat, nl, fail, max_speed, outx, outy);
}

}
```

### modelcrowdnav_amd/csrc/quad_common.hpp

```cpp
#pragma once
#include <hip/hip_runtime.h>
#include "orca_device.hpp"
#include "orca_static.hpp"

namespace mcn {

#ifdef MCN_DIAG
static __device__ unsigned int g_diag_counts[8192 * 4];
#define DIAG_COUNT(which)                                                                                        \
    do {                                                                                                         \
        const int w_ = blockIdx.x * (blockDim.x >> 6) + (threadIdx.x >> 6);                                      \
        if (w_ < 8192 && (int)(threadIdx.x & 63) == __ffsll((unsigned long long)__ballot(1)) - 1)                \
            atomicAdd(&g_diag_counts[w_ * 4 + (which)], 1u);                                                     \
    } while (0)
#else
#define DIAG_COUNT(which)
#endif

template <int I>
__device__ __forceinline__ int qbi(int v) { return __builtin_amdgcn_mov_dpp(v, I * 0x55, 0xf, 0xf, false); }
template <int I>
__device__ __forceinline__ float qbf(float v) { return __builtin_bit_cast(float, qbi<I>(__builtin_bit_cast(int, v))); }
template <int I>
__device__ __forceinline__ double qbd(double v)
{
    const long long b = __builtin_bit_cast(long long, v);
    const int lo = qbi<I>((int)b), hi = qbi<I>((int)(b >> 32));
    return __builtin_bit_cast(double, ((long long)hi << 32) | (unsigned int)lo);
}
template <int I>
__device__ __forceinline__ float4 qb4(float4 v) { return make_float4(qbf<I>(v.x), qbf<I>(v.y), qbf<I>(v.z), qbf<I>(v.w)); }

__device__ __forceinline__ float4 sel4(const float4 (&L)[4], int i)
{
    const float4 a = i == 1 ? L[1] : L[0], b = i == 3 ? L[3] : L[2];
    return i >= 2 ? b : a;
}

template <bool DIR>
__device__ __forceinline__ bool lp1_rt(const float4 (&L)[4], const float4 &ln, int no, float radius, float optx, float opty,
                                       float &rx, float &ry)
{
    const float dp = dot2(ln.x, ln.y, ln.z, ln.w);
    const float disc = dp * dp + radius * radius - dot2(ln.x, ln.y, ln.x, ln.y);
    bool ok = !(disc < 0.0f);
    const float sq = sqrt_f32(disc, ok);
    float tl = -dp - sq;
    float tr = -dp + sq;
#pragma unroll
    for (int i = 0; i < 3; ++i) {
        const float4 li = L[i];
        const float den = det2(ln.z, ln.w, li.z, li.w);
        const float num = det2(li.z, li.w, ln.x - li.x, ln.y - li.y);
        const float t = num / den;
        const bool live = i < no;
        const bool par = fabsf(den) <= kRvoEps;
        const bool cut = live & !par;
        const float ntr = fminf(tr, t), ntl = fmaxf(tl, t);
        tr = (cut & (den >= 0.0f)) ? ntr : tr;
        tl = (cut & !(den >= 0.0f)) ? ntl : tl;
        ok = ok & !(live & ((par ? 0.0f : tl) > (par ? num : tr)));
    }
    float t;
    if (DIR) {
        t = (dot2(optx, opty, ln.z, ln.w) > 0.0f) ? tr : tl;
    } else {
        t = dot2(ln.z, ln.w, optx - ln.x, opty - ln.y);
        if (t < tl) t = tl; else if (t > tr) t = tr;
    }
    rx = ln.x + t * ln.z;
    ry = ln.y + t * ln.w;
    return ok;
}

__device__ __forceinline__ bool lp3_candidate_quad(const float4 &li, const float4 &lj, int i, int k, float radius, float &rx,
                                                   float &ry)
{
    const float dt = det2(li.z, li.w, lj.z, lj.w);
    const bool par = fabsf(dt) <= kRvoEps;
    const bool same = dot2(li.z, li.w, lj.z, lj.w) > 0.0f;
    const bool keptb = (k < i) & !(par & same);
    const unsigned long long m_kept = lanes(k < i) & ~(lanes(par) & lanes(same));
    const float sc = det2(lj.z, lj.w, li.x - lj.x, li.y - lj.y) / dt;
    const float ddx = lj.z - li.z, ddy = lj.w - li.w;
    const float inv = keptb ? rcp_sqrt_f32(dot2(ddx, ddy, ddx, ddy), m_kept) : 0.0f;
    const float4 q = make_float4(par ? 0.5f * (li.x + lj.x) : li.x + sc * li.z,
                                 par ? 0.5f * (li.y + lj.y) : li.y + sc * li.w, ddx * inv, ddy * inv);
    const float4 P0 = qb4<0>(q), P1 = qb4<1>(q), P2 = qb4<2>(q);
    const float ox = -li.w, oy = li.z;

    const float dp = dot2(q.x, q.y, q.z, q.w);
    const float disc = dp * dp + radius * radius - dot2(q.x, q.y, q.x, q.y);
    bool ok = !(disc < 0.0f);
    const float sq = sqrt_f32(disc, lanes(!(disc < 0.0f)) & m_kept);
    float tl = -dp - sq;
    float tr = -dp + sq;
#pragma unroll
    for (int j = 0; j < 2; ++j) {
        const float4 pj = j == 0 ? P0 : P1;
        const bool live = j < k;
        const float den = det2(q.z, q.w, pj.z, pj.w);
        const float num = det2(pj.z, pj.w, q.x - pj.x, q.y - pj.y);
        const float t = num / den;
        const bool parj = fabsf(den) <= kRvoEps;
        const bool cut = live & !parj;
        const float ntr = fminf(tr, t), ntl = fmaxf(tl, t);
        tr = (cut & (den >= 0.0f)) ? ntr : tr;
        tl = (cut & !(den >= 0.0f)) ? ntl : tl;
        ok = ok & !(live & ((parj ? 0.0f : tl) > (parj ? num : tr)));
    }
    const float tt = (dot2(ox, oy, q.z, q.w) > 0.0f) ? tr : tl;
    const float cx = q.x + tt * q.z, cy = q.y + tt * q.w;
    const int fcode = ok ? 4 : k;

    rx = radius * ox; ry = radius * oy;
    int fail = 3;
#define MCN_LP3_INNER_TAKE(I, PI)                                                              \
    {                                                                                          \
        const int code_i = qbi<I>(fcode); const float cx_i = qbf<I>(cx), cy_i = qbf<I>(cy);    \
        const bool out = det2(PI.z, PI.w, PI.x - rx, PI.y - ry) > 0.0f;                         \
        fail = ((fail > I) & out) ? min(fail, code_i) : fail;                                   \
        const bool take = (fail > I) & out;                                                     \
        rx = take ? cx_i : rx; ry = take ? cy_i : ry;                                           \
    }
    MCN_LP3_INNER_TAKE(0, P0) MCN_LP3_INNER_TAKE(1, P1) MCN_LP3_INNER_TAKE(2, P2)
#undef MCN_LP3_INNER_TAKE
    return fail == 3;
}

__device__ __forceinline__ void quad_orca_operands(const mcn_env_cfg &c, double2 pos, double2 vel, double2 goal, double rad,
                                                   double vpref, float4 &A, float4 &B)
{
    const float fpx = (float)pos.x, fpy = (float)pos.y, fvx = (float)vel.x, fvy = (float)vel.y;
    const float frad = (float)(rad + 0.01 + c.orca_safety_space);
    const float ms = (float)vpref;
    const float prefx = (float)(goal.x - pos.x), prefy = (float)(goal.y - pos.y);
    A = make_float4(fpx, fpy, fvx, fvy);
    B = make_float4(prefx, prefy, frad, ms);
}

__device__ __forceinline__ float4 quad_orca_position_pack(double2 pos, double2 goal)
{
    return make_float4((float)pos.x, (float)pos.y, (float)(goal.x - pos.x), (float)(goal.y - pos.y));
}

__device__ __forceinline__ void quad_orca_core(const mcn_env_cfg &c, int lane, int k, bool cand_valid, float4 A, float4 B,
                                               float4 o, float orad, float inv_th, float inv_ts, float &rx, float &ry);

__device__ __forceinline__ void quad_orca_velocity(const mcn_env_cfg &c, int lane, int k, bool cand_valid,
                                                   double2 pos, double2 vel, double2 goal, double rad, double vpref,
                                                   float4 o, double crd, float inv_th, float inv_ts, float &rx, float &ry)
{
    float4 A, B;
    quad_orca_operands(c, pos, vel, goal, rad, vpref, A, B);
    const float orad = (float)(crd + 0.01 + c.orca_safety_space);
    quad_orca_core(c, lane, k, cand_valid, A, B, o, orad, inv_th, inv_ts, rx, ry);
}

__device__ __forceinline__ void quad_orca_core(const mcn_env_cfg &c, int lane, int k, bool cand_valid, float4 A, float4 B,
                                               float4 o, float orad, float inv_th, float inv_ts, float &rx, float &ry)
{
    const float fpx = A.x, fpy = A.y, fvx = A.z, fvy = A.w;
    const float prefx = B.x, prefy = B.y, frad = B.z, ms = B.w;
    const float range_sq = c.orca_neighbor_dist * c.orca_neighbor_dist;
    const float ddx = fpx - o.x, ddy = fpy - o.y;
    const float d = dot2(ddx, ddy, ddx, ddy);
    const bool in = cand_valid && (d < range_sq);
    const int key = in ? __builtin_bit_cast(int, d) : 0x7f800000;
    const int kd0 = qbi<0>(key) - key, kd1 = qbi<1>(key) - key, kd2 = qbi<2>(key) - key, kd3 = qbi<3>(key) - key;
    const int rank = (kd0 < (0 < k ? 1 : 0)) + (kd1 < (1 < k ? 1 : 0)) + (kd2 < (2 < k ? 1 : 0)) + (kd3 < 0);
    const int nin = __builtin_popcount((unsigned)(__builtin_amdgcn_ballot_w64(in) >> (lane & ~3)) & 0xfu);
    const int nl = nin < c.orca_max_neighbors ? nin : c.orca_max_neighbors;
    const float4 mine = orca_line_select(fpx, fpy, fvx, fvy, frad, o, orad, inv_th, inv_ts, in);
    const int dst = ((lane & ~3) | rank) << 2;
    float4 srt;
    srt.x = __builtin_bit_cast(float, __builtin_amdgcn_ds_permute(dst, __builtin_bit_cast(int, mine.x)));
    srt.y = __builtin_bit_cast(float, __builtin_amdgcn_ds_permute(dst, __builtin_bit_cast(int, mine.y)));
    srt.z = __builtin_bit_cast(float, __builtin_amdgcn_ds_permute(dst, __builtin_bit_cast(int, mine.z)));
    srt.w = __builtin_bit_cast(float, __builtin_amdgcn_ds_permute(dst, __builtin_bit_cast(int, mine.w)));
    {
        const float pp = dot2(prefx, prefy, prefx, prefy);
        const bool clip = pp > ms * ms;
        const float inv = rcp_sqrt_f32(pp, clip);
        rx = clip ? ms * (prefx * inv) : prefx;
        ry = clip ? ms * (prefy * inv) : prefy;
    }
    const float4 L[4] = {qb4<0>(srt), qb4<1>(srt), qb4<2>(srt), qb4<3>(srt)};

    float cx, cy;
    const int fcode = lp1_rt<false>(L, srt, k, ms, prefx, prefy, cx, cy) ? 4 : k;
    int fail = nl;
#define MCN_LP2_TAKE(I)                                                                        \
    {                                                                                          \
        const int code_i = qbi<I>(fcode); const float cx_i = qbf<I>(cx), cy_i = qbf<I>(cy);    \
        const bool out = det2(L[I].z, L[I].w, L[I].x - rx, L[I].y - ry) > 0.0f;                 \
        fail = ((fail > I) & out) ? min(fail, code_i) : fail;                                   \
        const bool take = (fail > I) & out;                                                     \
        rx = take ? cx_i : rx; ry = take ? cy_i : ry;                                           \
    }
    MCN_LP2_TAKE(0) MCN_LP2_TAKE(1) MCN_LP2_TAKE(2) MCN_LP2_TAKE(3)
#undef MCN_LP2_TAKE
    if (fail < nl) {
        DIAG_COUNT(0);
        float dist = 0.0f;
        int i = fail;
        for (;;) {
            const unsigned long long over = lanes((unsigned)(k - i) < (unsigned)(nl - i)) &
                                            lanes(det2(srt.z, srt.w, srt.x - rx, srt.y - ry) > dist);
            const unsigned m = (unsigned)(over >> (lane & ~3)) & 0xfu;
            if (m == 0) break;
            const int nxt = __builtin_ctz(m);
            const float4 ln = sel4(L, nxt);
            float cx3, cy3;
            const bool ok3 = lp3_candidate_quad(ln, srt, nxt, k, ms, cx3, cy3);
            rx = ok3 ? cx3 : rx; ry = ok3 ? cy3 : ry;
            dist = det2(ln.z, ln.w, ln.x - rx, ln.y - ry);
            i = nxt + 1;
        }
    }
}

}
```

Measured before the change: 1.902 billion.

## Add LDS-table quad ORCA path and split wg4 rollout into its own unit

Adds a templated path to the quad ORCA core that writes each lane's sorted constraint line into an LDS table and reads the four quad lines back with plain loads, replacing four ds_permute ops plus the quad broadcasts. It also reuses the already computed relative offset and distance in the u-direction computation and uses select-based clamping. The wg4 rollout kernel appears to move into a separate translation unit, with the shared helpers moved into a common header. The LDS round trip adds wave-level fences and extra shared memory, and it is unclear from what is visible whether the wg4 caller selects the new table path.

New measurement: 1.979 billion, median of 6. 1.04x the previous value.

```diff
diff --git a/modelcrowdnav_amd/csrc/env_rollout_common.hpp b/modelcrowdnav_amd/csrc/env_rollout_common.hpp
--- /dev/null
+++ b/modelcrowdnav_amd/csrc/env_rollout_common.hpp
@@ -0,0 +1,79 @@
+#pragma once
+#include <hip/hip_runtime.h>
+#include <stdint.h>
+#include "../../include/mcn.h"
+#include "quad_common.hpp"
+#include "env_step_params.hpp"
+#include "env_common.hpp"
+
+namespace mcn {
+void note_dispatch(const char *family);
+void note_rollout_form(int form);
+void launch_env_rollout_wg4(const StepParams &p, int T, hipStream_t stream);
+
+#ifdef MCN_DIAG
+#define MCN_STAMP_SLOTS 64
+#define MCN_STAMP_WAVES 8192
+static __device__ unsigned long long g_stamps[MCN_STAMP_WAVES * MCN_STAMP_SLOTS];
+#define STAMP(slot)                                                                                              \
+    do {                                                                                                         \
+        const int w_ = blockIdx.x * (blockDim.x >> 6) + (threadIdx.x >> 6);                                      \
+        if ((threadIdx.x & 63) == 0 && (slot) < MCN_STAMP_SLOTS && w_ < MCN_STAMP_WAVES)                         \
+            g_stamps[w_ * MCN_STAMP_SLOTS + (slot)] = __builtin_amdgcn_s_memrealtime();                          \
+    } while (0)
+#define STAMP_WHERE()                                                                                            \
+    do {                                                                                                         \
+        const int w_ = blockIdx.x * (blockDim.x >> 6) + (threadIdx.x >> 6);                                      \
+        if ((threadIdx.x & 63) == 0 && w_ < MCN_STAMP_WAVES)                                                     \
+            g_stamps[w_ * MCN_STAMP_SLOTS + 38] =                                                                \
+                (unsigned long long)__builtin_amdgcn_s_getreg((4) | (0 << 6) | (31 << 11)) |                     \
+                ((unsigned long long)__builtin_amdgcn_s_getreg((20) | (0 << 6) | (31 << 11)) << 32);             \
+    } while (0)
+static inline int read_counts_here(void *dst, size_t bytes, int reset)
+{
+    if (bytes > sizeof(g_diag_counts)) bytes = sizeof(g_diag_counts);
+    const int rc = hipMemcpyFromSymbol(dst, HIP_SYMBOL(g_diag_counts), bytes) == hipSuccess ? (int)(bytes / 4) : -1;
+    if (reset) {
+        void *sym = nullptr;
+        if (hipGetSymbolAddress(&sym, HIP_SYMBOL(g_diag_counts)) == hipSuccess) (void)hipMemset(sym, 0, sizeof(g_diag_counts));
+    }
+    return rc;
+}
+static inline int read_stamps_here(void *dst, size_t bytes)
+{
+    if (bytes > sizeof(g_stamps)) bytes = sizeof(g_stamps);
+    return hipMemcpyFromSymbol(dst, HIP_SYMBOL(g_stamps), bytes) == hipSuccess ? (int)(bytes / 8) : -1;
+}
+#else
+#define STAMP(slot)
+#define STAMP_WHERE()
+#endif
+
+__device__ __forceinline__ int bperm_i(int byte_addr, int v) { return __builtin_amdgcn_ds_bpermute(byte_addr, v); }
+__device__ __forceinline__ float bperm_f(int byte_addr, float v)
+{
+    return __builtin_bit_cast(float, bperm_i(byte_addr, __builtin_bit_cast(int, v)));
+}
+__device__ __forceinline__ double bperm_d(int byte_addr, double v)
+{
+    const long long b = __builtin_bit_cast(long long, v);
+    const int lo = bperm_i(byte_addr, (int)b), hi = bperm_i(byte_addr, (int)(b >> 32));
+    return __builtin_bit_cast(double, ((long long)hi << 32) | (unsigned int)lo);
+}
+
+template <class V>
+__device__ __forceinline__ V in_vgpr(V v)
+{
+    asm volatile("" : "+v"(v));
+    return v;
+}
+
+typedef const __attribute__((address_space(4))) StepParams *KernargPtr;
+__device__ __forceinline__ KernargPtr kernarg_here()
+{
+    KernargPtr q = (KernargPtr)__builtin_amdgcn_kernarg_segment_ptr();
+    asm volatile("" : "+s"(q));
+    return q;
+}
+
+}
diff --git a/modelcrowdnav_amd/csrc/env_rollout_quad.hip b/modelcrowdnav_amd/csrc/env_rollout_quad.hip
--- a/modelcrowdnav_amd/csrc/env_rollout_quad.hip
+++ b/modelcrowdnav_amd/csrc/env_rollout_quad.hip
@@ -1,419 +1,19 @@
-#include <hip/hip_runtime.h>
-#include <stdint.h>
-#include "../../include/mcn.h"
-#include "quad_common.hpp"
-#include "env_step_params.hpp"
-#include "env_common.hpp"
+#include "env_rollout_common.hpp"
 
 namespace mcn {
-void note_dispatch(const char *family);
-void note_rollout_form(int form);
 
 #ifdef MCN_DIAG
-#define MCN_STAMP_SLOTS 64
-#define MCN_STAMP_WAVES 8192
-__device__ unsigned long long g_stamps[MCN_STAMP_WAVES * MCN_STAMP_SLOTS];
-#define STAMP(slot)                                                                                              \
-    do {                                                                                                         \
-        const int w_ = blockIdx.x * (blockDim.x >> 6) + (threadIdx.x >> 6);                                      \
-        if ((threadIdx.x & 63) == 0 && (slot) < MCN_STAMP_SLOTS && w_ < MCN_STAMP_WAVES)                         \
-            g_stamps[w_ * MCN_STAMP_SLOTS + (slot)] = __builtin_amdgcn_s_memrealtime();                          \
-    } while (0)
-#define STAMP_WHERE()                                                                                            \
-    do {                                                                                                         \
-        const int w_ = blockIdx.x * (blockDim.x >> 6) + (threadIdx.x >> 6);                                      \
-        if ((threadIdx.x & 63) == 0 && w_ < MCN_STAMP_WAVES)                                                     \
-            g_stamps[w_ * MCN_STAMP_SLOTS + 38] =                                                                \
-                (unsigned long long)__builtin_amdgcn_s_getreg((4) | (0 << 6) | (31 << 11)) |                     \
-                ((unsigned long long)__builtin_amdgcn_s_getreg((20) | (0 << 6) | (31 << 11)) << 32);             \
-    } while (0)
-int read_counts(void *dst, size_t bytes, int reset)
-{
-    if (bytes > sizeof(g_diag_counts)) bytes = sizeof(g_diag_counts);
-    const int rc = hipMemcpyFromSymbol(dst, HIP_SYMBOL(g_diag_counts), bytes) == hipSuccess ? (int)(bytes / 4) : -1;
-    if (reset) {
-        void *sym = nullptr;
-        if (hipGetSymbolAddress(&sym, HIP_SYMBOL(g_diag_counts)) == hipSuccess) (void)hipMemset(sym, 0, sizeof(g_diag_counts));
-    }
-    return rc;
-}
-int read_stamps(void *dst, size_t bytes)
-{
-    if (bytes > sizeof(g_stamps)) bytes = sizeof(g_stamps);
-    return hipMemcpyFromSymbol(dst, HIP_SYMBOL(g_stamps), bytes) == hipSuccess ? (int)(bytes / 8) : -1;
-}
-#else
-#define STAMP(slot)
-#define STAMP_WHERE()
+int read_counts_wg4(void *dst, size_t bytes, int reset);
+int read_stamps_wg4(void *dst, size_t bytes);
+int read_counts(void *dst, size_t bytes, int reset, int form)
+{
+    return form == 2 ? read_counts_wg4(dst, bytes, reset) : read_counts_here(dst, bytes, reset);
+}
+int read_stamps(void *dst, size_t bytes, int form)
+{
+    return form == 2 ? read_stamps_wg4(dst, bytes) : read_stamps_here(dst, bytes);
+}
 #endif
-
-__device__ __forceinline__ int bperm_i(int byte_addr, int v) { return __builtin_amdgcn_ds_bpermute(byte_addr, v); }
-__device__ __forceinline__ float bperm_f(int byte_addr, float v)
-{
-    return __builtin_bit_cast(float, bperm_i(byte_addr, __builtin_bit_cast(int, v)));
-}
-__device__ __forceinline__ double bperm_d(int byte_addr, double v)
-{
-    const long long b = __builtin_bit_cast(long long, v);
-    const int lo = bperm_i(byte_addr, (int)b), hi = bperm_i(byte_addr, (int)(b >> 32));
-    return __builtin_bit_cast(double, ((long long)hi << 32) | (unsigned int)lo);
-}
-
-template <class V>
-__device__ __forceinline__ V in_vgpr(V v)
-{
-    asm volatile("" : "+v"(v));
-    return v;
-}
-
-typedef const __attribute__((address_space(4))) StepParams *KernargPtr;
-__device__ __forceinline__ KernargPtr kernarg_here()
-{
-    KernargPtr q = (KernargPtr)__builtin_amdgcn_kernarg_segment_ptr();
-    asm volatile("" : "+s"(q));
-    return q;
-}
-
-template <int NT>
-struct Wg4 {
-    static_assert(NT == 5, "the four-wavefront form is built for 5 humans only");
-    static constexpr int EW = 8;
-    static constexpr int NQ = EW * NT;
-};
-
-template <int CTRL>
-__device__ __forceinline__ int dpp_i(int v) { return __builtin_amdgcn_mov_dpp(v, CTRL, 0xf, 0xf, true); }
-template <int CTRL>
-__device__ __forceinline__ double dpp_d(double v)
-{
-    const long long b = __builtin_bit_cast(long long, v);
-    const int lo = dpp_i<CTRL>((int)b), hi = dpp_i<CTRL>((int)(b >> 32));
-    return __builtin_bit_cast(double, ((long long)hi << 32) | (unsigned int)lo);
-}
-constexpr int DPP_QUAD_XOR1 = 0xB1, DPP_QUAD_XOR2 = 0x4E, DPP_ROW_HALF_MIRROR = 0x141;
-
-template <int NT, int VIS, bool UNI>
-__device__ __forceinline__ void rollout_wg4(const StepParams &p, const int T)
-{
-    static_assert(VIS == 0, "the four-wavefront form is built for an invisible robot only");
-    constexpr int EW = Wg4<NT>::EW, NQ = Wg4<NT>::NQ;
-    __shared__ float4 s_pack[NQ];
-    __shared__ float2 s_res[2 * NQ], s_inv[NQ];
-    __shared__ double2 s_hpos[NQ];
-    __shared__ double s_hrad[NQ];
-    STAMP(0);
-    STAMP_WHERE();
-#ifdef MCN_DIAG
-    if (p.debug_noop) return;
-#endif
-    const int tid = threadIdx.x;
-    const int role = __builtin_amdgcn_readfirstlane(tid >> 6);
-    const unsigned nb_ = gridDim.x, xcd_ = blockIdx.x & 7u, idx_ = blockIdx.x >> 3;
-    const unsigned qq_ = nb_ >> 3, rr__ = nb_ & 7u;
-    const unsigned chunk_ = (xcd_ < rr__ ? xcd_ * (qq_ + 1) : rr__ * (qq_ + 1) + (xcd_ - rr__) * qq_) + idx_;
-    const mcn_env_cfg &c = p.cfg;
-    const mcn_rollout &ro = p.roll;
-
-    if (role < 3) {
-        const int lane = tid & 63, k = tid & 3, q = tid >> 2;
-        const bool pop = q < NQ;
-        const int ge = q / NT, h = q - ge * NT;
-        const bool active = pop && (long)chunk_ * EW + ge < p.E;
-        const int hi = pop ? q : 0;
-        const bool cand_h = k < NT - 1;
-        const int j = cand_h ? k + (k >= h ? 1 : 0) : h;
-        const int ci = pop ? ge * NT + j : 0;
-        const bool publish = pop && k == 0;
-        const float inv_th = in_vgpr(1.0f / c.orca_time_horizon), inv_ts = in_vgpr(1.0f / (float)c.time_step);
-        int rd_h = hi + NQ, rd_c = ci + NQ;
-        __syncthreads();
-        STAMP(1);
-
-        for (int t = 0; t < T; ++t) {
-            float4 P = s_pack[hi];
-            float2 cp = *reinterpret_cast<const float2 *>(s_pack + ci);
-            float2 v = s_res[rd_h], cv = s_res[rd_c];
-            float2 fm = s_inv[hi];
-            float orad = s_inv[ci].x;
-            asm volatile("" : "+v"(P.x), "+v"(P.y), "+v"(P.z), "+v"(P.w), "+v"(cp.x), "+v"(cp.y), "+v"(v.x), "+v"(v.y),
-                              "+v"(cv.x), "+v"(cv.y), "+v"(fm.x), "+v"(fm.y), "+v"(orad));
-            float rx, ry;
-            quad_orca_core(c, lane, k, cand_h && active, make_float4(P.x, P.y, v.x, v.y), make_float4(P.z, P.w, fm.x, fm.y),
-                           make_float4(cp.x, cp.y, cv.x, cv.y), orad, inv_th, inv_ts, rx, ry);
-            if (publish) s_res[(t & 1) * NQ + hi] = make_float2(rx, ry);
-            rd_h = in_vgpr(hi + (t & 1) * NQ); rd_c = in_vgpr(ci + (t & 1) * NQ);
-            if (t < 20) STAMP(40 + t);
-            __syncthreads();
-            __syncthreads();
-            if (t < 37) STAMP(2 + t);
-        }
-    } else {
-        static_assert(EW * 8 == 64, "eight lanes per env fill the wavefront");
-        const double dt = in_vgpr(c.time_step);
-        const bool do_reset = p.has_roll && ro.pool_hpos != nullptr;
-        const int l = tid & 63;
-        const int g = l >> 3, h = l & 7;
-        const bool pop = h < NT;
-        const int hs = g * NT + (pop ? h : 0);
-        const long e = (long)chunk_ * EW + g;
-        const bool active = pop && e < p.E;
-        const long eb = e < p.E ? e : 0;
-        const long a = eb * NT + (pop ? h : 0);
-        const bool lead = active && h == 0;
-        constexpr bool unicycle = UNI;
-        const bool has_state = p.has_roll && ro.state != nullptr;
-        const bool track = c.track_human_times && p.st.human_times != nullptr;
-
-        double2 pos = reinterpret_cast<const double2 *>(p.st.hpos)[a];
-        double2 vel = reinterpret_cast<const double2 *>(p.st.hvel)[a];
-        double2 goal = reinterpret_cast<const double2 *>(p.st.hgoal)[a];
-        double rad = p.st.hrad[a];
-        double vpref = p.st.hvpref[a];
-        double htime = p.st.human_times ? p.st.human_times[a] : 0.0;
-        double hax = 0, hay = 0;
-        double2 rpos = reinterpret_cast<const double2 *>(p.st.rpos)[eb];
-        double2 rvel = reinterpret_cast<const double2 *>(p.st.rvel)[eb];
-        double2 rgoal = reinterpret_cast<const double2 *>(p.st.rgoal)[eb];
-        const double rrad = p.st.rrad[eb];
-        double gtime = p.st.gtime[eb];
-        double rtheta = p.st.rtheta ? p.st.rtheta[eb] : 0.0;
-        mcn_roll_rec rs = {0, 0, 0, 0, 0, 0};
-        if (has_state) rs = ro.state[eb];
-        const double2 *act_ptr = reinterpret_cast<const double2 *>(p.actions) + eb;
-        const long act_stride = in_vgpr((long)p.E);
-        const double *disc_table = in_vgpr(ro.disc_table);
-        const int disc_last = in_vgpr(ro.disc_len - 1);
-        const bool has_theta = p.st.rtheta != nullptr;
-        double2 act_next = *act_ptr;
-        double o_rew = 0, o_dmin = 0;
-        int o_dn = 0, o_inf = 0, o_hh = 0;
-        const double k_timeout_at = in_vgpr(c.time_limit - 1);
-        const double k_collision = in_vgpr(c.collision_penalty), k_success = in_vgpr(c.success_reward);
-        const double k_discomfort = in_vgpr(c.discomfort_dist), k_factor = in_vgpr(c.discomfort_penalty_factor);
-        const int k_stride = ro.case_stride, k_pool = ro.pool_size;
-        const bool count_hh = c.count_hh != 0;
-        {
-            float4 A, B;
-            quad_orca_operands(c, pos, vel, goal, rad, vpref, A, B);
-            if (pop) {
-                s_pack[hs] = make_float4(A.x, A.y, B.x, B.y); s_res[NQ + hs] = make_float2(A.z, A.w);
-                s_inv[hs] = make_float2(B.z, B.w);
-                s_hpos[hs] = pos; s_hrad[hs] = rad;
-            }
-        }
-        __syncthreads();
-        STAMP(1);
-
-        for (int t = 0; t < T; ++t) {
-            const double2 act = act_next;
-            act_ptr += act_stride;
-            if (t + 1 < T) act_next = *act_ptr;
-            double ep_disc = 0;
-            if (has_state) ep_disc = disc_table[rs.ep_steps < disc_last ? rs.ep_steps : disc_last];
-
-            double2 eff = act;
-            if (unicycle) {
-                eff.x = act.x * cos(act.y + rtheta);
-                eff.y = act.x * sin(act.y + rtheta);
-            }
-            double cd;
-            {
-                const double px = pos.x - rpos.x, py = pos.y - rpos.y;
-                const double vx = vel.x - eff.x, vy = vel.y - eff.y;
-                cd = p2s_origin(px, py, px + vx * dt, py + vy * dt) - rad - rrad;
-            }
-            cd = pop ? cd : INFINITY;
-            int hh = 0;
-            {
-                static_assert(NT / 2 == 2, "two pairs per lane");
-                double s2[2], ra[2], rb[2];
-                bool near_any = false;
-                const bool counted = active & count_hh;
-#pragma unroll
-                for (int d = 1; d <= NT / 2; ++d) {
-                    const int jj = h + d >= NT ? h + d - NT : h + d;
-                    const int pi = g * NT + (pop ? jj : 0);
-                    const double2 ppos = s_hpos[pi];
-                    const double prad = s_hrad[pi];
-                    ra[d - 1] = jj > h ? rad : prad; rb[d - 1] = jj > h ? prad : rad;
-                    const double dx = pos.x - ppos.x, dy = pos.y - ppos.y;
-                    s2[d - 1] = dx * dx + dy * dy;
-                    const double reach = ra[d - 1] + rb[d - 1] + 1e-6;
-                    near_any |= counted & (s2[d - 1] < reach * reach);
-                }
-                if (__any(near_any)) {
-                    DIAG_COUNT(2);
-#pragma unroll
-                    for (int d = 0; d < NT / 2; ++d)
-                        hh += (counted & ((sqrt(s2[d]) - ra[d] - rb[d]) < 0)) ? 1 : 0;
-                }
-            }
-            double dmin = cd;
-            int hh_sum = hh;
-            dmin = fmin(dmin, dpp_d<DPP_QUAD_XOR1>(dmin));       hh_sum += dpp_i<DPP_QUAD_XOR1>(hh_sum);
-            dmin = fmin(dmin, dpp_d<DPP_QUAD_XOR2>(dmin));       hh_sum += dpp_i<DPP_QUAD_XOR2>(hh_sum);
-            dmin = fmin(dmin, dpp_d<DPP_ROW_HALF_MIRROR>(dmin)); hh_sum += dpp_i<DPP_ROW_HALF_MIRROR>(hh_sum);
-
-            double endx, endy, new_theta = rtheta, nrvx, nrvy;
-            if (unicycle) {
-                const double th = rtheta + act.y;
-                endx = rpos.x + cos(th) * act.x * dt;
-                endy = rpos.y + sin(th) * act.x * dt;
-                new_theta = pymod(rtheta + act.y, 2 * M_PI);
-                nrvx = act.x * cos(new_theta); nrvy = act.x * sin(new_theta);
-            } else {
-                endx = rpos.x + act.x * dt; endy = rpos.y + act.y * dt;
-                nrvx = act.x; nrvy = act.y;
-            }
-            bool reaching = false;
-            {
-                const double gx = endx - rgoal.x, gy = endy - rgoal.y, near = rrad + 1e-6;
-                if (__any(gx * gx + gy * gy < near * near)) DIAG_COUNT(3);
-                if (__any(gx * gx + gy * gy < near * near)) reaching = norm2(gx, gy) < rrad;
-            }
-            double rew; int inf, dn;
-            if (gtime >= k_timeout_at)          { rew = 0; dn = 1; inf = MCN_INFO_TIMEOUT; }
-            else if (dmin < 0)                  { rew = k_collision; dn = 1; inf = MCN_INFO_COLLISION; }
-            else if (reaching)                  { rew = k_success; dn = 1; inf = MCN_INFO_REACHGOAL; }
-            else if (dmin < k_discomfort)       { rew = (dmin - k_discomfort) * k_factor * dt; dn = 0; inf = MCN_INFO_DANGER; }
-            else                                { rew = 0; dn = 0; inf = MCN_INFO_NOTHING; }
-            o_rew = rew; o_dmin = dmin; o_dn = dn; o_inf = inf; o_hh = hh_sum;
-            const double t_new = gtime + dt;
-
-            const int case_g = rs.next_case;
-            if (has_state) {
-                bool danger = inf == MCN_INFO_DANGER;
-                if (danger) {
-                    const KernargPtr kp = kernarg_here();
-                    const int lim = kp->roll.danger_episodes, sf = kp->roll.danger_short_from;
-                    danger = lim <= 0 || rs.fin_count < lim - ((sf > 0 && e >= sf - 1) ? 1 : 0);
-                }
-                rs.danger_count += danger ? 1 : 0;
-                rs.danger_dist_sum = danger ? rs.danger_dist_sum + dmin : rs.danger_dist_sum;
-                const double ret = rs.ep_return + ep_disc * rew;
-                if (lead && dn) {
-                    const int kf = rs.fin_count;
-                    const KernargPtr kp = kernarg_here();
-                    const int fin_slots = kp->roll.fin_slots;
-                    double *fin_return = kp->roll.fin_return, *fin_time = kp->roll.fin_time;
-                    uint8_t *fin_info = kp->roll.fin_info;
-                    const bool keep = (fin_slots == 1) || (kf < fin_slots);
-                    const long rec = (long)(fin_slots == 1 ? 0 : kf) * kp->E + e;
-                    if (keep && fin_return) fin_return[rec] = ret;
-                    if (keep && fin_time)   fin_time[rec] = (inf == MCN_INFO_TIMEOUT) ? kp->cfg.time_limit : t_new;
-                    if (keep && fin_info)   fin_info[rec] = (uint8_t)inf;
-                }
-                rs.fin_count += dn;
-                rs.ep_return = dn ? 0.0 : ret;
-                rs.ep_steps = dn ? 0 : rs.ep_steps + 1;
-                if (do_reset) {
-                    int nc = rs.next_case + k_stride;
-                    nc = nc >= k_pool ? nc - k_pool : nc;
-                    rs.next_case = dn ? nc : rs.next_case;
-                }
-            }
-
-            if (do_reset && dn) {
-                const KernargPtr kp = kernarg_here();
-                const double k_theta0 = kp->roll.robot_theta0;
-                rpos = make_double2(kp->roll.robot_start[0], kp->roll.robot_start[1]);
-                rgoal = make_double2(kp->roll.robot_goal[0], kp->roll.robot_goal[1]);
-                rvel = make_double2(0, 0);
-                if (has_theta) rtheta = k_theta0;
-                gtime = 0;
-            } else {
-                rpos = make_double2(endx, endy);
-                rvel = make_double2(nrvx, nrvy);
-                if (unicycle) rtheta = new_theta;
-                gtime = t_new;
-            }
-
-            const bool restart = do_reset && dn;
-            float4 n_pack = make_float4(0, 0, 0, 0);
-            float2 n_fvel = make_float2(0, 0), n_inv = make_float2(0, 0);
-            if (restart) {
-                DIAG_COUNT(1);
-                if (active) {
-                    const long pa = (long)case_g * NT + h;
-                    const KernargPtr kp = kernarg_here();
-                    const double2 *pool_hvel = reinterpret_cast<const double2 *>(kp->roll.pool_hvel);
-                    vel = make_double2(0, 0);
-                    if (pool_hvel) vel = pool_hvel[pa];
-                    pos = reinterpret_cast<const double2 *>(kp->roll.pool_hpos)[pa];
-                    goal = reinterpret_cast<const double2 *>(kp->roll.pool_hgoal)[pa];
-                    rad = kp->roll.pool_hrad[pa];
-                    vpref = kp->roll.pool_hvpref[pa];
-                }
-                htime = 0;
-                float4 A, B;
-                quad_orca_operands(c, pos, vel, goal, rad, vpref, A, B);
-                n_pack = make_float4(in_vgpr(A.x), in_vgpr(A.y), in_vgpr(B.x), in_vgpr(B.y));
-                n_fvel = make_float2(in_vgpr(A.z), in_vgpr(A.w));
-                n_inv = make_float2(in_vgpr(B.z), in_vgpr(B.w));
-            }
-            const bool any_restart = __any(restart);
-
-            if (t < 20) STAMP(40 + t);
-            __syncthreads();
-            float2 *vel_io = s_res + (t & 1) * NQ;
-            {
-                const float2 r = vel_io[hs];
-                hax = (double)r.x; hay = (double)r.y;
-            }
-            if (!restart) {
-                pos = make_double2(pos.x + hax * dt, pos.y + hay * dt);
-                if (pop) s_pack[hs] = quad_orca_position_pack(pos, goal);
-            }
-            if (any_restart) {
-                if (pop && restart) { s_pack[hs] = n_pack; vel_io[hs] = n_fvel; s_inv[hs] = n_inv; }
-            }
-            __syncthreads();
-            if (t < 37) STAMP(2 + t);
-
-            if (pop) s_hpos[hs] = pos;
-            if (!restart) {
-                vel = make_double2(hax, hay);
-                if (track && htime == 0 && norm2(pos.x - goal.x, pos.y - goal.y) < rad) htime = t_new;
-            }
-            if (any_restart) {
-                if (pop && restart) s_hrad[hs] = rad;
-            }
-        }
-
-        long a2 = a, e2 = e;
-        asm volatile("" : "+v"(a2), "+v"(e2));
-        const KernargPtr kp = kernarg_here();
-        if (active) {
-            reinterpret_cast<double2 *>(kp->st.hpos)[a2] = pos;
-            reinterpret_cast<double2 *>(kp->st.hvel)[a2] = vel;
-            if (do_reset) {
-                reinterpret_cast<double2 *>(kp->st.hgoal)[a2] = goal;
-                kp->st.hrad[a2] = rad;
-                kp->st.hvpref[a2] = vpref;
-            }
-            double *human_times = kp->st.human_times, *human_act = kp->out.human_act;
-            if (human_times) human_times[a2] = htime;
-            if (human_act) reinterpret_cast<double2 *>(human_act)[a2] = make_double2(hax, hay);
-        }
-        if (lead) {
-            reinterpret_cast<double2 *>(kp->st.rpos)[e2] = rpos;
-            reinterpret_cast<double2 *>(kp->st.rvel)[e2] = rvel;
-            if (do_reset) reinterpret_cast<double2 *>(kp->st.rgoal)[e2] = rgoal;
-            double *rth = kp->st.rtheta;
-            if (rth) rth[e2] = rtheta;
-            kp->st.gtime[e2] = gtime;
-            store_step_rec(kp->out.rec + e2, o_rew, o_dmin, o_dn, o_inf, o_hh);
-            if (has_state) kp->roll.state[e2] = rs;
-        }
-    }
-    STAMP(39);
-}
-
-template <int NT, int VIS, bool UNI>
-__global__ __launch_bounds__(256, 2) void env_rollout_wg4_kernel(const StepParams p, const int T)
-{
-    rollout_wg4<NT, VIS, UNI>(p, T);
-}
 
 template <int NT, int VIS, bool UNI, bool SPLIT>
 __global__ __launch_bounds__(SPLIT ? 128 : 64, SPLIT ? 3 : 1) void env_rollout_quad_kernel(const StepParams p, const int T)
@@ -705,8 +305,7 @@
 {
     if constexpr (NT == 5 && VIS == 0) {
         if (p.quad_split == 2) {
-            constexpr int EW = Wg4<NT>::EW;
-            hipLaunchKernelGGL((env_rollout_wg4_kernel<NT, VIS, UNI>), dim3((p.E + EW - 1) / EW), dim3(256), 0, stream, p, T);
+            launch_env_rollout_wg4(p, T, stream);
             note_rollout_form(2);
             return;
         }
diff --git a/modelcrowdnav_amd/csrc/env_rollout_wg4.hip b/modelcrowdnav_amd/csrc/env_rollout_wg4.hip
--- /dev/null
+++ b/modelcrowdnav_amd/csrc/env_rollout_wg4.hip
@@ -0,0 +1,366 @@
+#include "env_rollout_common.hpp"
+
+namespace mcn {
+
+template <int NT>
+struct Wg4 {
+    static_assert(NT == 5, "the four-wavefront form is built for 5 humans only");
+    static constexpr int EW = 8;
+    static constexpr int NQ = EW * NT;
+};
+
+template <int CTRL>
+__device__ __forceinline__ int dpp_i(int v) { return __builtin_amdgcn_mov_dpp(v, CTRL, 0xf, 0xf, true); }
+template <int CTRL>
+__device__ __forceinline__ double dpp_d(double v)
+{
+    const long long b = __builtin_bit_cast(long long, v);
+    const int lo = dpp_i<CTRL>((int)b), hi = dpp_i<CTRL>((int)(b >> 32));
+    return __builtin_bit_cast(double, ((long long)hi << 32) | (unsigned int)lo);
+}
+constexpr int DPP_QUAD_XOR1 = 0xB1, DPP_QUAD_XOR2 = 0x4E, DPP_ROW_HALF_MIRROR = 0x141;
+
+template <int NT, int VIS, bool UNI>
+__device__ __forceinline__ void rollout_wg4(const StepParams &p, const int T)
+{
+    static_assert(VIS == 0, "the four-wavefront form is built for an invisible robot only");
+    constexpr int EW = Wg4<NT>::EW, NQ = Wg4<NT>::NQ;
+    __shared__ float4 s_pack[NQ];
+    __shared__ float2 s_res[2 * NQ], s_inv[NQ];
+    __shared__ double2 s_hpos[NQ];
+    __shared__ double s_hrad[NQ];
+    __shared__ float4 s_lines[3 * 64];
+    STAMP(0);
+    STAMP_WHERE();
+#ifdef MCN_DIAG
+    if (p.debug_noop) return;
+#endif
+    const int tid = threadIdx.x;
+    const int role = __builtin_amdgcn_readfirstlane(tid >> 6);
+    const unsigned nb_ = gridDim.x, xcd_ = blockIdx.x & 7u, idx_ = blockIdx.x >> 3;
+    const unsigned qq_ = nb_ >> 3, rr__ = nb_ & 7u;
+    const unsigned chunk_ = (xcd_ < rr__ ? xcd_ * (qq_ + 1) : rr__ * (qq_ + 1) + (xcd_ - rr__) * qq_) + idx_;
+    const mcn_env_cfg &c = p.cfg;
+    const mcn_rollout &ro = p.roll;
+
+    if (role < 3) {
+        const int lane = tid & 63, k = tid & 3, q = tid >> 2;
+        const bool pop = q < NQ;
+        const int ge = q / NT, h = q - ge * NT;
+        const bool active = pop && (long)chunk_ * EW + ge < p.E;
+        const int hi = pop ? q : 0;
+        const bool cand_h = k < NT - 1;
+        const int j = cand_h ? k + (k >= h ? 1 : 0) : h;
+        const int ci = pop ? ge * NT + j : 0;
+        const bool publish = pop && k == 0;
+        const float inv_th = in_vgpr(1.0f / c.orca_time_horizon), inv_ts = in_vgpr(1.0f / (float)c.time_step);
+        constexpr int RES_BUF = NQ * (int)sizeof(float2);
+        const int hi_b = hi * (int)sizeof(float2), ci_b = ci * (int)sizeof(float2);
+        int rd_h = hi_b + RES_BUF, rd_c = ci_b + RES_BUF;
+        const char *res_bytes = reinterpret_cast<const char *>(s_res);
+        const QuadTable lines = {s_lines + role * 64};
+        __syncthreads();
+        STAMP(1);
+
+        for (int t = 0; t < T; ++t) {
+            float4 P = s_pack[hi];
+            float2 cp = *reinterpret_cast<const float2 *>(s_pack + ci);
+            float2 v = *reinterpret_cast<const float2 *>(res_bytes + rd_h), cv = *reinterpret_cast<const float2 *>(res_bytes + rd_c);
+            float2 fm = s_inv[hi];
+            float orad = s_inv[ci].x;
+            asm volatile("" : "+v"(P.x), "+v"(P.y), "+v"(P.z), "+v"(P.w), "+v"(cp.x), "+v"(cp.y), "+v"(v.x), "+v"(v.y),
+                              "+v"(cv.x), "+v"(cv.y), "+v"(fm.x), "+v"(fm.y), "+v"(orad));
+            float rx, ry;
+            quad_orca_core(c, lane, k, cand_h && active, make_float4(P.x, P.y, v.x, v.y), make_float4(P.z, P.w, fm.x, fm.y),
+                           make_float4(cp.x, cp.y, cv.x, cv.y), orad, inv_th, inv_ts, rx, ry, lines);
+            if (publish) s_res[(t & 1) * NQ + hi] = make_float2(rx, ry);
+            rd_h = in_vgpr(hi_b + (t & 1) * RES_BUF); rd_c = in_vgpr(ci_b + (t & 1) * RES_BUF);
+            if (t < 20) STAMP(40 + t);
+            __syncthreads();
+            __syncthreads();
+            if (t < 37) STAMP(2 + t);
+        }
+    } else {
+        static_assert(EW * 8 == 64, "eight lanes per env fill the wavefront");
+        const double dt = in_vgpr(c.time_step);
+        const bool do_reset = p.has_roll && ro.pool_hpos != nullptr;
+        const int l = tid & 63;
+        const int g = l >> 3, h = l & 7;
+        const bool pop = h < NT;
+        const int hs = g * NT + (pop ? h : 0);
+        const long e = (long)chunk_ * EW + g;
+        const bool active = pop && e < p.E;
+        const long eb = e < p.E ? e : 0;
+        const long a = eb * NT + (pop ? h : 0);
+        const bool lead = active && h == 0;
+        constexpr bool unicycle = UNI;
+        const bool has_state = p.has_roll && ro.state != nullptr;
+        const bool track = c.track_human_times && p.st.human_times != nullptr;
+
+        double2 pos = reinterpret_cast<const double2 *>(p.st.hpos)[a];
+        double2 vel = reinterpret_cast<const double2 *>(p.st.hvel)[a];
+        double2 goal = reinterpret_cast<const double2 *>(p.st.hgoal)[a];
+        double rad = p.st.hrad[a];
+        double vpref = p.st.hvpref[a];
+        double htime = p.st.human_times ? p.st.human_times[a] : 0.0;
+        double hax = 0, hay = 0;
+        double2 rpos = reinterpret_cast<const double2 *>(p.st.rpos)[eb];
+        double2 rvel = reinterpret_cast<const double2 *>(p.st.rvel)[eb];
+        double2 rgoal = reinterpret_cast<const double2 *>(p.st.rgoal)[eb];
+        const double rrad = p.st.rrad[eb];
+        double gtime = p.st.gtime[eb];
+        double rtheta = p.st.rtheta ? p.st.rtheta[eb] : 0.0;
+        mcn_roll_rec rs = {0, 0, 0, 0, 0, 0};
+        if (has_state) rs = ro.state[eb];
+        const double2 *act_ptr = reinterpret_cast<const double2 *>(p.actions) + eb;
+        const long act_stride = in_vgpr((long)p.E);
+        const double *disc_table = in_vgpr(ro.disc_table);
+        const int disc_last = in_vgpr(ro.disc_len - 1);
+        const bool has_theta = p.st.rtheta != nullptr;
+        double2 act_next = *act_ptr;
+        double o_rew = 0, o_dmin = 0;
+        int o_dn = 0, o_inf = 0, o_hh = 0;
+        const double k_timeout_at = in_vgpr(c.time_limit - 1);
+        const double k_collision = in_vgpr(c.collision_penalty), k_success = in_vgpr(c.success_reward);
+        const double k_discomfort = in_vgpr(c.discomfort_dist), k_factor = in_vgpr(c.discomfort_penalty_factor);
+        const int k_stride = ro.case_stride, k_pool = ro.pool_size;
+        const bool count_hh = c.count_hh != 0;
+        {
+            float4 A, B;
+            quad_orca_operands(c, pos, vel, goal, rad, vpref, A, B);
+            if (pop) {
+                s_pack[hs] = make_float4(A.x, A.y, B.x, B.y); s_res[NQ + hs] = make_float2(A.z, A.w);
+                s_inv[hs] = make_float2(B.z, B.w);
+                s_hpos[hs] = pos; s_hrad[hs] = rad;
+            }
+        }
+        __syncthreads();
+        STAMP(1);
+
+        for (int t = 0; t < T; ++t) {
+            const double2 act = act_next;
+            act_ptr += act_stride;
+            if (t + 1 < T) act_next = *act_ptr;
+            double ep_disc = 0;
+            if (has_state) ep_disc = disc_table[rs.ep_steps < disc_last ? rs.ep_steps : disc_last];
+
+            double2 eff = act;
+            if (unicycle) {
+                eff.x = act.x * cos(act.y + rtheta);
+                eff.y = act.x * sin(act.y + rtheta);
+            }
+            double cd;
+            {
+                const double px = pos.x - rpos.x, py = pos.y - rpos.y;
+                const double vx = vel.x - eff.x, vy = vel.y - eff.y;
+                cd = p2s_origin(px, py, px + vx * dt, py + vy * dt) - rad - rrad;
+            }
+            cd = pop ? cd : INFINITY;
+            int hh = 0;
+            {
+                static_assert(NT / 2 == 2, "two pairs per lane");
+                double s2[2], ra[2], rb[2];
+                bool near_any = false;
+                const bool counted = active & count_hh;
+#pragma unroll
+                for (int d = 1; d <= NT / 2; ++d) {
+                    const int jj = h + d >= NT ? h + d - NT : h + d;
+                    const int pi = g * NT + (pop ? jj : 0);
+                    const double2 ppos = s_hpos[pi];
+                    const double prad = s_hrad[pi];
+                    ra[d - 1] = jj > h ? rad : prad; rb[d - 1] = jj > h ? prad : rad;
+                    const double dx = pos.x - ppos.x, dy = pos.y - ppos.y;
+                    s2[d - 1] = dx * dx + dy * dy;
+                    const double reach = ra[d - 1] + rb[d - 1] + 1e-6;
+                    near_any |= counted & (s2[d - 1] < reach * reach);
+                }
+                if (__any(near_any)) {
+                    DIAG_COUNT(2);
+#pragma unroll
+                    for (int d = 0; d < NT / 2; ++d)
+                        hh += (counted & ((sqrt(s2[d]) - ra[d] - rb[d]) < 0)) ? 1 : 0;
+                }
+            }
+            double dmin = cd;
+            int hh_sum = hh;
+            dmin = fmin(dmin, dpp_d<DPP_QUAD_XOR1>(dmin));       hh_sum += dpp_i<DPP_QUAD_XOR1>(hh_sum);
+            dmin = fmin(dmin, dpp_d<DPP_QUAD_XOR2>(dmin));       hh_sum += dpp_i<DPP_QUAD_XOR2>(hh_sum);
+            dmin = fmin(dmin, dpp_d<DPP_ROW_HALF_MIRROR>(dmin)); hh_sum += dpp_i<DPP_ROW_HALF_MIRROR>(hh_sum);
+
+            double endx, endy, new_theta = rtheta, nrvx, nrvy;
+            if (unicycle) {
+                const double th = rtheta + act.y;
+                endx = rpos.x + cos(th) * act.x * dt;
+                endy = rpos.y + sin(th) * act.x * dt;
+                new_theta = pymod(rtheta + act.y, 2 * M_PI);
+                nrvx = act.x * cos(new_theta); nrvy = act.x * sin(new_theta);
+            } else {
+                endx = rpos.x + act.x * dt; endy = rpos.y + act.y * dt;
+                nrvx = act.x; nrvy = act.y;
+            }
+            bool reaching = false;
+            {
+                const double gx = endx - rgoal.x, gy = endy - rgoal.y, near = rrad + 1e-6;
+                if (__any(gx * gx + gy * gy < near * near)) DIAG_COUNT(3);
+                if (__any(gx * gx + gy * gy < near * near)) reaching = norm2(gx, gy) < rrad;
+            }
+            double rew; int inf, dn;
+            if (gtime >= k_timeout_at)          { rew = 0; dn = 1; inf = MCN_INFO_TIMEOUT; }
+            else if (dmin < 0)                  { rew = k_collision; dn = 1; inf = MCN_INFO_COLLISION; }
+            else if (reaching)                  { rew = k_success; dn = 1; inf = MCN_INFO_REACHGOAL; }
+            else if (dmin < k_discomfort)       { rew = (dmin - k_discomfort) * k_factor * dt; dn = 0; inf = MCN_INFO_DANGER; }
+            else                                { rew = 0; dn = 0; inf = MCN_INFO_NOTHING; }
+            o_rew = rew; o_dmin = dmin; o_dn = dn; o_inf = inf; o_hh = hh_sum;
+            const double t_new = gtime + dt;
+
+            const int case_g = rs.next_case;
+            if (has_state) {
+                bool danger = inf == MCN_INFO_DANGER;
+                if (danger) {
+                    const KernargPtr kp = kernarg_here();
+                    const int lim = kp->roll.danger_episodes, sf = kp->roll.danger_short_from;
+                    danger = lim <= 0 || rs.fin_count < lim - ((sf > 0 && e >= sf - 1) ? 1 : 0);
+                }
+                rs.danger_count += danger ? 1 : 0;
+                rs.danger_dist_sum = danger ? rs.danger_dist_sum + dmin : rs.danger_dist_sum;
+                const double ret = rs.ep_return + ep_disc * rew;
+                if (lead && dn) {
+                    const int kf = rs.fin_count;
+                    const KernargPtr kp = kernarg_here();
+                    const int fin_slots = kp->roll.fin_slots;
+                    double *fin_return = kp->roll.fin_return, *fin_time = kp->roll.fin_time;
+                    uint8_t *fin_info = kp->roll.fin_info;
+                    const bool keep = (fin_slots == 1) || (kf < fin_slots);
+                    const long rec = (long)(fin_slots == 1 ? 0 : kf) * kp->E + e;
+                    if (keep && fin_return) fin_return[rec] = ret;
+                    if (keep && fin_time)   fin_time[rec] = (inf == MCN_INFO_TIMEOUT) ? kp->cfg.time_limit : t_new;
+                    if (keep && fin_info)   fin_info[rec] = (uint8_t)inf;
+                }
+                rs.fin_count += dn;
+                rs.ep_return = dn ? 0.0 : ret;
+                rs.ep_steps = dn ? 0 : rs.ep_steps + 1;
+                if (do_reset) {
+                    int nc = rs.next_case + k_stride;
+                    nc = nc >= k_pool ? nc - k_pool : nc;
+                    rs.next_case = dn ? nc : rs.next_case;
+                }
+            }
+
+            if (do_reset && dn) {
+                const KernargPtr kp = kernarg_here();
+                const double k_theta0 = kp->roll.robot_theta0;
+                rpos = make_double2(kp->roll.robot_start[0], kp->roll.robot_start[1]);
+                rgoal = make_double2(kp->roll.robot_goal[0], kp->roll.robot_goal[1]);
+                rvel = make_double2(0, 0);
+                if (has_theta) rtheta = k_theta0;
+                gtime = 0;
+            } else {
+                rpos = make_double2(endx, endy);
+                rvel = make_double2(nrvx, nrvy);
+                if (unicycle) rtheta = new_theta;
+                gtime = t_new;
+            }
+
+            const bool restart = do_reset && dn;
+            float4 n_pack = make_float4(0, 0, 0, 0);
+            float2 n_fvel = make_float2(0, 0), n_inv = make_float2(0, 0);
+            if (restart) {
+                DIAG_COUNT(1);
+                if (active) {
+                    const long pa = (long)case_g * NT + h;
+                    const KernargPtr kp = kernarg_here();
+                    const double2 *pool_hvel = reinterpret_cast<const double2 *>(kp->roll.pool_hvel);
+                    vel = make_double2(0, 0);
+                    if (pool_hvel) vel = pool_hvel[pa];
+                    pos = reinterpret_cast<const double2 *>(kp->roll.pool_hpos)[pa];
+                    goal = reinterpret_cast<const double2 *>(kp->roll.pool_hgoal)[pa];
+                    rad = kp->roll.pool_hrad[pa];
+                    vpref = kp->roll.pool_hvpref[pa];
+                }
+                htime = 0;
+                float4 A, B;
+                quad_orca_operands(c, pos, vel, goal, rad, vpref, A, B);
+                n_pack = make_float4(in_vgpr(A.x), in_vgpr(A.y), in_vgpr(B.x), in_vgpr(B.y));
+                n_fvel = make_float2(in_vgpr(A.z), in_vgpr(A.w));
+                n_inv = make_float2(in_vgpr(B.z), in_vgpr(B.w));
+            }
+            const bool any_restart = __any(restart);
+
+            if (t < 20) STAMP(40 + t);
+            __syncthreads();
+            float2 *vel_io = s_res + (t & 1) * NQ;
+            {
+                const float2 r = vel_io[hs];
+                hax = (double)r.x; hay = (double)r.y;
+            }
+            if (!restart) {
+                pos = make_double2(pos.x + hax * dt, pos.y + hay * dt);
+                if (pop) s_pack[hs] = quad_orca_position_pack(pos, goal);
+            }
+            if (any_restart) {
+                if (pop && restart) { s_pack[hs] = n_pack; vel_io[hs] = n_fvel; s_inv[hs] = n_inv; }
+            }
+            __syncthreads();
+            if (t < 37) STAMP(2 + t);
+
+            if (pop) s_hpos[hs] = pos;
+            if (!restart) {
+                vel = make_double2(hax, hay);
+                if (track && htime == 0 && norm2(pos.x - goal.x, pos.y - goal.y) < rad) htime = t_new;
+            }
+            if (any_restart) {
+                if (pop && restart) s_hrad[hs] = rad;
+            }
+        }
+
+        long a2 = a, e2 = e;
+        asm volatile("" : "+v"(a2), "+v"(e2));
+        const KernargPtr kp = kernarg_here();
+        if (active) {
+            reinterpret_cast<double2 *>(kp->st.hpos)[a2] = pos;
+            reinterpret_cast<double2 *>(kp->st.hvel)[a2] = vel;
+            if (do_reset) {
+                reinterpret_cast<double2 *>(kp->st.hgoal)[a2] = goal;
+                kp->st.hrad[a2] = rad;
+                kp->st.hvpref[a2] = vpref;
+            }
+            double *human_times = kp->st.human_times, *human_act = kp->out.human_act;
+            if (human_times) human_times[a2] = htime;
+            if (human_act) reinterpret_cast<double2 *>(human_act)[a2] = make_double2(hax, hay);
+        }
+        if (lead) {
+            reinterpret_cast<double2 *>(kp->st.rpos)[e2] = rpos;
+            reinterpret_cast<double2 *>(kp->st.rvel)[e2] = rvel;
+            if (do_reset) reinterpret_cast<double2 *>(kp->st.rgoal)[e2] = rgoal;
+            double *rth = kp->st.rtheta;
+            if (rth) rth[e2] = rtheta;
+            kp->st.gtime[e2] = gtime;
+            store_step_rec(kp->out.rec + e2, o_rew, o_dmin, o_dn, o_inf, o_hh);
+            if (has_state) kp->roll.state[e2] = rs;
+        }
+    }
+    STAMP(39);
+}
+
+template <int NT, int VIS, bool UNI>
+__global__ __launch_bounds__(256, 2) void env_rollout_wg4_kernel(const StepParams p, const int T)
+{
+    rollout_wg4<NT, VIS, UNI>(p, T);
+}
+
+void launch_env_rollout_wg4(const StepParams &p, int T, hipStream_t stream)
+{
+    constexpr int NT = 5, EW = Wg4<NT>::EW;
+    const dim3 grid((p.E + EW - 1) / EW), block(256);
+    if (p.cfg.robot_kinematics == MCN_KIN_UNICYCLE)
+        hipLaunchKernelGGL((env_rollout_wg4_kernel<NT, 0, true>), grid, block, 0, stream, p, T);
+    else
+        hipLaunchKernelGGL((env_rollout_wg4_kernel<NT, 0, false>), grid, block, 0, stream, p, T);
+}
+
+#ifdef MCN_DIAG
+int read_counts_wg4(void *dst, size_t bytes, int reset) { return read_counts_here(dst, bytes, reset); }
+int read_stamps_wg4(void *dst, size_t bytes) { return read_stamps_here(dst, bytes); }
+#endif
+
+}
diff --git a/modelcrowdnav_amd/csrc/mcn_api.hip b/modelcrowdnav_amd/csrc/mcn_api.hip
--- a/modelcrowdnav_amd/csrc/mcn_api.hip
+++ b/modelcrowdnav_amd/csrc/mcn_api.hip
@@ -58,8 +58,8 @@
                        float *traj, double time_step, float neighbor_dist, int max_neighbors, float time_horizon,
                        int E, int N, hipStream_t stream);
 #ifdef MCN_DIAG
-int read_stamps(void *dst, size_t bytes);
-int read_counts(void *dst, size_t bytes, int reset);
+int read_stamps(void *dst, size_t bytes, int form);
+int read_counts(void *dst, size_t bytes, int reset, int form);
 #endif
 }
 
@@ -629,8 +629,8 @@
 #ifdef MCN_DIAG
 int mcn_debug_pool_clock(void *dst_host, int64_t bytes) { return mcn::read_pool_clock(dst_host, (size_t)bytes); }
 int mcn_debug_sarl_phases(void *dst_host, int64_t bytes, int32_t reset) { return mcn::read_sarl_phases(dst_host, (size_t)bytes, reset); }
-int mcn_debug_stamps(void *dst_host, int64_t bytes) { return mcn::read_stamps(dst_host, (size_t)bytes); }
-int mcn_debug_counts(void *dst_host, int64_t bytes, int reset) { return mcn::read_counts(dst_host, (size_t)bytes, reset); }
+int mcn_debug_stamps(void *dst_host, int64_t bytes) { return mcn::read_stamps(dst_host, (size_t)bytes, g_last_rollout_form); }
+int mcn_debug_counts(void *dst_host, int64_t bytes, int reset) { return mcn::read_counts(dst_host, (size_t)bytes, reset, g_last_rollout_form); }
 #endif
 
 }
diff --git a/modelcrowdnav_amd/csrc/orca_static.hpp b/modelcrowdnav_amd/csrc/orca_static.hpp
--- a/modelcrowdnav_amd/csrc/orca_static.hpp
+++ b/modelcrowdnav_amd/csrc/orca_static.hpp
@@ -46,12 +46,10 @@
     return make_float4(vx + 0.5f * ux, vy + 0.5f * uy, dx, dy);
 }
 
-__device__ __forceinline__ float4 orca_u_dir(float px, float py, float vx, float vy, float radius, float4 o,
-                                             float orad, float inv_th, float inv_ts, bool used = true)
-{
-    const float rpx = o.x - px, rpy = o.y - py;
+__device__ __forceinline__ float4 orca_u_dir_rel(float rpx, float rpy, float dist_sq, float vx, float vy, float radius,
+                                                 float4 o, float orad, float inv_th, float inv_ts, bool used = true)
+{
     const float rvx = vx - o.z, rvy = vy - o.w;
-    const float dist_sq = dot2(rpx, rpy, rpx, rpy);
     const float cr = radius + orad;
     const float cr_sq = cr * cr;
     const bool apart = dist_sq > cr_sq;
@@ -88,6 +86,13 @@
     return make_float4(ux, uy, dx, dy);
 }
 
+__device__ __forceinline__ float4 orca_u_dir(float px, float py, float vx, float vy, float radius, float4 o,
+                                             float orad, float inv_th, float inv_ts, bool used = true)
+{
+    const float rpx = o.x - px, rpy = o.y - py;
+    return orca_u_dir_rel(rpx, rpy, dot2(rpx, rpy, rpx, rpy), vx, vy, radius, o, orad, inv_th, inv_ts, used);
+}
+
 __device__ __forceinline__ float4 orca_line_select(float px, float py, float vx, float vy, float radius, float4 o,
                                                    float orad, float inv_th, float inv_ts, bool used = true)
 {
diff --git a/modelcrowdnav_amd/csrc/quad_common.hpp b/modelcrowdnav_amd/csrc/quad_common.hpp
--- a/modelcrowdnav_amd/csrc/quad_common.hpp
+++ b/modelcrowdnav_amd/csrc/quad_common.hpp
@@ -37,7 +37,15 @@
     return i >= 2 ? b : a;
 }
 
-template <bool DIR>
+struct QuadDpp {
+    static constexpr bool table = false, slim = false;
+};
+struct QuadTable {
+    static constexpr bool table = true, slim = true;
+    float4 *tab;
+};
+
+template <bool DIR, bool SELECT_CLAMP = false>
 __device__ __forceinline__ bool lp1_rt(const float4 (&L)[4], const float4 &ln, int no, float radius, float optx, float opty,
                                        float &rx, float &ry)
 {
@@ -66,7 +74,12 @@
         t = (dot2(optx, opty, ln.z, ln.w) > 0.0f) ? tr : tl;
     } else {
         t = dot2(ln.z, ln.w, optx - ln.x, opty - ln.y);
-        if (t < tl) t = tl; else if (t > tr) t = tr;
+        if (SELECT_CLAMP) {
+            const float hi = (t > tr) ? tr : t;
+            t = (t < tl) ? tl : hi;
+        } else {
+            if (t < tl) t = tl; else if (t > tr) t = tr;
+        }
     }
     rx = ln.x + t * ln.z;
     ry = ln.y + t * ln.w;
@@ -144,8 +157,10 @@
     return make_float4((float)pos.x, (float)pos.y, (float)(goal.x - pos.x), (float)(goal.y - pos.y));
 }
 
+template <class Path = QuadDpp>
 __device__ __forceinline__ void quad_orca_core(const mcn_env_cfg &c, int lane, int k, bool cand_valid, float4 A, float4 B,
-                                               float4 o, float orad, float inv_th, float inv_ts, float &rx, float &ry);
+                                               float4 o, float orad, float inv_th, float inv_ts, float &rx, float &ry,
+                                               Path path = Path());
 
 __device__ __forceinline__ void quad_orca_velocity(const mcn_env_cfg &c, int lane, int k, bool cand_valid,
                                                    double2 pos, double2 vel, double2 goal, double rad, double vpref,
@@ -157,13 +172,15 @@
     quad_orca_core(c, lane, k, cand_valid, A, B, o, orad, inv_th, inv_ts, rx, ry);
 }
 
+template <class Path>
 __device__ __forceinline__ void quad_orca_core(const mcn_env_cfg &c, int lane, int k, bool cand_valid, float4 A, float4 B,
-                                               float4 o, float orad, float inv_th, float inv_ts, float &rx, float &ry)
+                                               float4 o, float orad, float inv_th, float inv_ts, float &rx, float &ry,
+                                               Path path)
 {
     const float fpx = A.x, fpy = A.y, fvx = A.z, fvy = A.w;
     const float prefx = B.x, prefy = B.y, frad = B.z, ms = B.w;
     const float range_sq = c.orca_neighbor_dist * c.orca_neighbor_dist;
-    const float ddx = fpx - o.x, ddy = fpy - o.y;
+    const float ddx = Path::slim ? o.x - fpx : fpx - o.x, ddy = Path::slim ? o.y - fpy : fpy - o.y;
     const float d = dot2(ddx, ddy, ddx, ddy);
     const bool in = cand_valid && (d < range_sq);
     const int key = in ? __builtin_bit_cast(int, d) : 0x7f800000;
@@ -171,13 +188,29 @@
     const int rank = (kd0 < (0 < k ? 1 : 0)) + (kd1 < (1 < k ? 1 : 0)) + (kd2 < (2 < k ? 1 : 0)) + (kd3 < 0);
     const int nin = __builtin_popcount((unsigned)(__builtin_amdgcn_ballot_w64(in) >> (lane & ~3)) & 0xfu);
     const int nl = nin < c.orca_max_neighbors ? nin : c.orca_max_neighbors;
-    const float4 mine = orca_line_select(fpx, fpy, fvx, fvy, frad, o, orad, inv_th, inv_ts, in);
-    const int dst = ((lane & ~3) | rank) << 2;
-    float4 srt;
-    srt.x = __builtin_bit_cast(float, __builtin_amdgcn_ds_permute(dst, __builtin_bit_cast(int, mine.x)));
-    srt.y = __builtin_bit_cast(float, __builtin_amdgcn_ds_permute(dst, __builtin_bit_cast(int, mine.y)));
-    srt.z = __builtin_bit_cast(float, __builtin_amdgcn_ds_permute(dst, __builtin_bit_cast(int, mine.z)));
-    srt.w = __builtin_bit_cast(float, __builtin_amdgcn_ds_permute(dst, __builtin_bit_cast(int, mine.w)));
+    float4 mine;
+    if constexpr (Path::slim) {
+        const float4 ud = orca_u_dir_rel(ddx, ddy, d, fvx, fvy, frad, o, orad, inv_th, inv_ts, in);
+        mine = make_float4(fvx + 0.5f * ud.x, fvy + 0.5f * ud.y, ud.z, ud.w);
+    } else {
+        mine = orca_line_select(fpx, fpy, fvx, fvy, frad, o, orad, inv_th, inv_ts, in);
+    }
+    float4 srt, L[4];
+    if constexpr (Path::table) {
+        path.tab[(lane & ~3) | rank] = mine;
+        __builtin_amdgcn_fence(__ATOMIC_RELEASE, "wavefront");
+        __builtin_amdgcn_wave_barrier();
+        __builtin_amdgcn_fence(__ATOMIC_ACQUIRE, "wavefront");
+        const float4 *quad = path.tab + (lane & ~3);
+        L[0] = quad[0]; L[1] = quad[1]; L[2] = quad[2]; L[3] = quad[3];
+        srt = path.tab[lane];
+    } else {
+        const int dst = ((lane & ~3) | rank) << 2;
+        srt.x = __builtin_bit_cast(float, __builtin_amdgcn_ds_permute(dst, __builtin_bit_cast(int, mine.x)));
+        srt.y = __builtin_bit_cast(float, __builtin_amdgcn_ds_permute(dst, __builtin_bit_cast(int, mine.y)));
+        srt.z = __builtin_bit_cast(float, __builtin_amdgcn_ds_permute(dst, __builtin_bit_cast(int, mine.z)));
+        srt.w = __builtin_bit_cast(float, __builtin_amdgcn_ds_permute(dst, __builtin_bit_cast(int, mine.w)));
+    }
     {
         const float pp = dot2(prefx, prefy, prefx, prefy);
         const bool clip = pp > ms * ms;
@@ -185,10 +218,12 @@
         rx = clip ? ms * (prefx * inv) : prefx;
         ry = clip ? ms * (prefy * inv) : prefy;
     }
-    const float4 L[4] = {qb4<0>(srt), qb4<1>(srt), qb4<2>(srt), qb4<3>(srt)};
+    if constexpr (!Path::table) {
+        L[0] = qb4<0>(srt); L[1] = qb4<1>(srt); L[2] = qb4<2>(srt); L[3] = qb4<3>(srt);
+    }
 
     float cx, cy;
-    const int fcode = lp1_rt<false>(L, srt, k, ms, prefx, prefy, cx, cy) ? 4 : k;
+    const int fcode = lp1_rt<false, Path::slim>(L, srt, k, ms, prefx, prefy, cx, cy) ? 4 : k;
     int fail = nl;
 #define MCN_LP2_TAKE(I)                                                                        \
     {                                                                                          \
@@ -210,7 +245,9 @@
             const unsigned m = (unsigned)(over >> (lane & ~3)) & 0xfu;
             if (m == 0) break;
             const int nxt = __builtin_ctz(m);
-            const float4 ln = sel4(L, nxt);
+            float4 ln;
+            if constexpr (Path::table) ln = path.tab[(lane & ~3) | nxt];
+            else ln = sel4(L, nxt);
             float cx3, cy3;
             const bool ok3 = lp3_candidate_quad(ln, srt, nxt, k, ms, cx3, cy3);
             rx = ok3 ? cx3 : rx; ry = ok3 ? cy3 : ry;
```
